# haosulab/ActiveZero

Hardware: AMD Instinct MI355X
Metric: stereo pairs/sec (540x960, D=192) fwd+bwd (higher is better)
Workload: dtype f32; 1 GPU; configs[1]: PSMNet 540x960 (padded to 544 rows) D=192 fwd+bwd+Adam, supervised disparity loss, batch 4 per GPU; global_batch=4, height=540, width=960, maxdisp=192, parallelism=dp1

## Files before the change

activezero_amd/conv3d.py:

```python
import collections
import os

import torch

from . import _lib, overlap, packing, profiler
from .amax import AMAX_SLOTS, ZEROS, absmax, _get_amax, _set_amax, weight_amax
from .handover import slot_contribute, slot_leftover, slot_register, sum_parts
from .ops import _call, _chk, _p, _stream

CONV_S1, CONV_S2, DECONV_S2 = 0, 1, 2
FP32, BF16X6, F16X3 = 0, 1, 3
_PREC = {"fp32": FP32, "bf16x6": BF16X6, "f16x3": F16X3}
_BWD_F16 = os.environ.get("AZ_BWD_F16", "1") != "0"
PRESPLIT = os.environ.get("AZ_PRESPLIT", "1") != "0"
BF16X6_R16 = 2
_ROLL = os.environ.get("AZ_CONV_ROLL", "1") != "0"


_OFF32 = 0xffffff00


def _fits32(x, cin, cout):
    if isinstance(x, LazyCostVolume):
        return True
    _, d, h, w, _ = x.shape
    return d * h * w * max(cin, cout) * 4 < _OFF32


def _fits32_transposed(x, op_cin, op_cout):
    if not (op_cin == 64 and op_cout == 32):
        return True
    _, d, h, w, _ = x.shape
    return d * h * w * 64 * 4 < _OFF32 and 8 * d * h * w * 32 * 4 < _OFF32


def _layout(precision, mode, op_cout, fits32=True):
    if precision == BF16X6 and mode == CONV_S1 and op_cout == 32 and _ROLL and fits32:
        return BF16X6_R16
    return precision


def _fwd_launch(weight, mode):
    if mode == DECONV_S2:
        cin, cout = weight.shape[0], weight.shape[1]
        return cin, cout, 27, cout * 27
    cout, cin = weight.shape[0], weight.shape[1]
    return cin, cout, cin * 27, 27


def _dgrad_launch(mode, cin, cout):
    if mode == CONV_S1:
        return CONV_S1, cout, cin, 27, cin * 27, True
    if mode == CONV_S2:
        return DECONV_S2, cout, cin, 27, cin * 27, False
    return CONV_S2, cout, cin, cout * 27, 27, False


def _f16_fwd_ok(mode, cin, cout):
    return cin in (32, 64) and cout in (32, 64)


def _f16_dgrad_ok(mode, cin, cout):
    return _f16_fwd_ok(*_dgrad_launch(mode, cin, cout)[:3])


def _f16_wgrad_ok(mode, cin, cout):
    return cin in (32, 64) and cout in (32, 64)


def _f16_launch_ok(op_mode, ci, co, operand):
    if not _f16_fwd_ok(op_mode, ci, co):
        return False
    if op_mode == DECONV_S2:
        return _fits32_transposed(operand, ci, co)
    if _fits32(operand, ci, co):
        return True
    if op_mode == CONV_S1:
        return not (co == 32 or ci == co == 64)
    return not (ci == 32 and co == 64 and _lib.lib().az_option(b"AZ_CONV_S2ROLL") != 0)


class Arith(collections.namedtuple("Arith", "conv wgrad sink bwd16", defaults=(None, False))):
    __slots__ = ()

    @classmethod
    def of(cls, conv="bf16x6", wgrad=None, bwd16=None):
        w = wgrad if wgrad is not None else conv
        if bwd16 is None:
            bwd16 = _BWD_F16 or conv == "f16x3"
        return cls(_PREC[conv], BF16X6 if w == "f16x3" else _PREC[w], None, bool(bwd16) and conv != "fp32" and w != "fp32")

    @property
    def names(self):
        inv = {v: k for k, v in _PREC.items()}
        return inv[self.conv], ("f16x3" if self.bwd16 else inv[self.wgrad])


DEFAULT_ARITH = Arith.of(os.environ.get("AZ_CONV_PRECISION", "f16x3"), os.environ.get("AZ_WGRAD_PRECISION"))


def _arith(a):
    if a is None:
        return DEFAULT_ARITH
    if isinstance(a, str):
        return Arith.of(a)
    return a


def _dims(x):
    b, d, h, w, c = x.shape
    return b, d, h, w, c


def _out_dims(mode, d, h, w):
    if mode == CONV_S1:
        return d, h, w
    if mode == CONV_S2:
        return (d - 1) // 2 + 1, (h - 1) // 2 + 1, (w - 1) // 2 + 1
    return 2 * d, 2 * h, 2 * w


def _pack(weight, op_cin, op_cout, stride_out, stride_in, flip, precision, cache=False):
    w = _chk(weight.detach().contiguous(), "weight")

    def make():
        n = _lib.lib().az_conv3d_packed_floats(op_cin, op_cout, precision)
        packed = torch.empty(n, dtype=torch.float32, device=w.device)
        _call("az_conv3d_pack_weights", _p(packed), _p(w), op_cin, op_cout, stride_out, stride_in,
              int(flip), precision, _stream())
        packed.az_precision = precision
        return packed

    key = (packing.cache_key(weight), op_cin, op_cout, stride_out, stride_in, bool(flip), precision) if cache else None
    return packing.memo(packing.PACK_CACHE, key, make, (weight,), 256)


def eval_affine(bn, like, cache=False):
    c = bn.num_features
    src = (bn.weight, bn.bias, bn.running_mean, bn.running_var, bn.num_batches_tracked)

    def make():
        scale, shift = like.new_empty(c), like.new_empty(c)
        _call("az_bn3d_eval_affine", _p(scale), _p(shift), _p(bn.weight.detach()), _p(bn.bias.detach()),
              _p(bn.running_mean), _p(bn.running_var), float(bn.eps), c, _stream())
        return scale, shift

    return packing.memo(packing.AFFINE_CACHE, (packing.cache_key(*src), float(bn.eps)) if cache else None, make, src, 512)


def _pack_forward(weight, mode, precision, cache=False, lazy=False, fits32=True):
    cin, cout, s_out, s_in = _fwd_launch(weight, mode)
    if not lazy:
        precision = _layout(precision, mode, cout, fits32)
    return _pack(weight, cin, cout, s_out, s_in, False, precision, cache), cin, cout


def _peak(precision):
    if precision == F16X3:
        return _PEAK_F16
    return (157.3, "fp32 MFMA") if precision == FP32 else (2500.0 / 6.0, "bf16x6: bf16 MFMA peak / 6")


def _conv_flops(b, vox_out, cin, cout, mode):
    taps = 27.0 / 8.0 if mode == DECONV_S2 else 27.0
    return 2.0 * taps * cin * cout * b * vox_out


class LazyCostVolume:

    def __init__(self, feat_l_nhwc, feat_r_nhwc, ndisp):
        self.fl, self.fr, self.ndisp = _chk(feat_l_nhwc, "feat_l"), _chk(feat_r_nhwc, "feat_r"), int(ndisp)
        if self.fl.shape != self.fr.shape or self.fl.shape[-1] != 32:
            raise RuntimeError("fused cost volume expects two [B,h,w,32] feature maps")


def _run_gather(x, packed, mode, cin, cout, precision, scale=None, shift=None, residual=None, relu=False,
                stats=False, tag="conv3d"):
    if isinstance(x, LazyCostVolume):
        if stats or mode != CONV_S1 or cin != 64:
            raise RuntimeError("the fused cost-volume operand is only wired for the eval-mode dres0[0] conv")
        b, h, w, _ = x.fl.shape
        d = x.ndisp
        out = x.fl.new_empty(b, d, h, w, cout)
        with profiler.scope(f"{tag}_costvol_m0_{cin}_{cout}", flops=_conv_flops(b, d * h * w, cin, cout, mode),
                            peak=_peak(precision)):
            _call("az_conv3d_fwd", _p(out), _p(x.fl), _p(x.fr), _p(packed), _p(scale), _p(shift),
                  _p(residual), int(relu), mode, 1, getattr(packed, "az_precision", precision), b, cin, cout, d, h, w,
                  _stream())
        return out
    b, d, h, w, c = _dims(x)
    assert c == cin, (c, cin)
    precision = getattr(packed, "az_precision", precision)
    if mode == CONV_S2 and ((d % 2 and d != 1) or h % 2 or w % 2):
        raise RuntimeError("stride-2 layers need even D/H/W (as PSMNet's hourglass does; D = 1: a 2-D layer)")
    do, ho, wo = _out_dims(mode, d, h, w)
    out = x.new_empty(b, do, ho, wo, cout)
    flops = _conv_flops(b, do * ho * wo, cin, cout, mode)
    name = f"{tag}_m{mode}_{cin}_{cout}"
    if stats:
        ntiles = _lib.lib().az_conv3d_stats_tiles(mode, precision, b, cin, cout, d, h, w)
        if ntiles <= 0:
            raise RuntimeError(f"az_conv3d_stats_tiles: {ntiles}")
        part = x.new_empty(cout, ntiles, 2)
        cnt = x.new_empty(ntiles)
        with profiler.scope(name, flops=flops, peak=_peak(precision)):
            _call("az_conv3d_fwd_stats", _p(out), _p(part), _p(cnt), _p(x), None, _p(packed), mode, 0,
                  precision, b, cin, cout, d, h, w, _stream())
        return out, part, cnt, ntiles
    with profiler.scope(name, flops=flops, peak=_peak(precision)):
        _call("az_conv3d_fwd", _p(out), _p(x), None, _p(packed), _p(scale), _p(shift), _p(residual),
              int(relu), mode, 0, precision, b, cin, cout, d, h, w, _stream())
    return out


_PEAK_F16 = (2500.0 / 3.0, "f16x3: fp16 MFMA peak / 3")


def _pack_f16(weight, op_cin, op_cout, stride_out, stride_in, flip, mode, cache=False):
    w = _chk(weight.detach().contiguous(), "weight")

    def pack_now(packed, w_amax):
        _call("az_conv3d_pack_weights_f16", _p(packed), _p(w), _p(w_amax), op_cin, op_cout, stride_out, stride_in,
              int(flip), mode, _stream())

    def make():
        w_amax = weight_amax(weight, w)
        packed = torch.empty(_lib.lib().az_conv3d_packed_floats_f16(op_cin, op_cout), dtype=torch.float32, device=w.device)
        pack_now(packed, w_amax)
        return packed, w_amax

    if cache:
        key = (packing.cache_key(weight), op_cin, op_cout, stride_out, stride_in, bool(flip), F16X3, mode)
        return packing.memo(packing.PACK_CACHE, key, make, (weight,), 256)
    kind = _lib.lib().az_conv3d_f16_layout(mode, op_cin, op_cout)
    if kind < 0:
        raise RuntimeError(f"az_conv3d_f16_layout({mode}, {op_cin}, {op_cout}): {kind}")
    hit = packing.planned_pack(weight, w, kind, op_cin, op_cout, op_cin, op_cout, stride_out, stride_in, 27, flip, pack_now)
    return hit if hit is not None else make()


def _is_split(t):
    return getattr(t, "az_split", False)


def _run_f16(x, packed, w_amax, mode, cin, cout, scale=None, shift=None, residual=None, relu=False, stats=False,
             tag="conv3d"):
    b, d, h, w, c = _dims(x)
    assert c == cin, (c, cin)
    do, ho, wo = _out_dims(mode, d, h, w)
    out = x.new_empty(b, do, ho, wo, cout)
    name = f"{tag}_m{mode}_{cin}_{cout}"
    flops = _conv_flops(b, do * ho * wo, cin, cout, mode)
    split = _is_split(x)
    x_amax = _get_amax(x) if split else absmax(x)
    if split and (stats or x_amax is None):
        raise RuntimeError("a pre-split tensor reached a launch that cannot read it")
    if stats:
        ntiles = _lib.lib().az_conv3d_stats_tiles_f16(mode, b, cin, cout, d, h, w)
        if ntiles <= 0:
            raise RuntimeError(f"az_conv3d_stats_tiles_f16: {ntiles}")
        part, cnt = x.new_empty(cout, ntiles, 2), x.new_empty(ntiles)
        with profiler.scope(name, flops=flops, peak=_PEAK_F16):
            _call("az_conv3d_fwd_stats_f16", _p(out), _p(part), _p(cnt), _p(x), _p(packed), _p(x_amax), _p(w_amax),
                  mode, b, cin, cout, d, h, w, _stream())
        return out, part, cnt, ntiles
    with profiler.scope(name, flops=flops, peak=_PEAK_F16):
        _call("az_conv3d_fwd_f16", _p(out), _p(x), _p(packed), _p(x_amax), _p(w_amax), int(split), _p(scale), _p(shift),
              _p(residual), int(relu), mode, b, cin, cout, d, h, w, _stream())
    return out


def _conv(x, weight, mode, precision, scale=None, shift=None, residual=None, relu=False, stats=False, cache=False,
          tag="conv3d"):
    lazy = isinstance(x, LazyCostVolume)
    cin, cout, s_out, s_in = _fwd_launch(weight, mode)
    if precision == F16X3 and not lazy and _f16_launch_ok(mode, cin, cout, x):
        pk, w_amax = _pack_f16(weight, cin, cout, s_out, s_in, False, mode, cache)
        return _run_f16(x, pk, w_amax, mode, cin, cout, scale, shift, residual, relu, stats, tag)
    prec = BF16X6 if precision == F16X3 else precision
    packed, cin, cout = _pack_forward(weight, mode, prec, cache=cache, lazy=lazy, fits32=_fits32(x, cin, cout))
    return _run_gather(x, packed, mode, cin, cout, prec, scale, shift, residual, relu, stats, tag)


def _wgrad_f16(coarse, fine, stride, cm, cn, tag, sink=None, late_ok=True):
    b, dc, hc, wc, _ = _dims(coarse)
    _, df, hf, wf, _ = _dims(fine)
    gw = coarse.new_empty(cm, cn, 3, 3, 3)
    ws_bytes = _lib.lib().az_conv3d_wgrad_workspace(cm, cn)
    am_c, am_f = _get_amax(coarse), _get_amax(fine)
    mask = (1 if _is_split(coarse) else 0) | (2 if _is_split(fine) else 0)
    if (mask & 1 and am_c is None) or (mask & 2 and am_f is None):
        raise RuntimeError("a pre-split tensor without its producer's amax")
    with overlap.scope(sink, coarse, fine, gw, am_c, am_f):
        late = late_ok and sink is not None and sink.live and overlap.DEFER_UNPACK
        ws = sink.take_workspace(ws_bytes // 4) if late else coarse.new_empty(ws_bytes // 4)
        am_c = am_c if mask & 1 else absmax(coarse)
        am_f = am_f if mask & 2 else absmax(fine)
        with profiler.scope(f"{tag}_wgrad_s{stride}_{cm}_{cn}", flops=2.0 * 27 * cm * cn * b * dc * hc * wc,
                            peak=_PEAK_F16):
            _call("az_conv3d_wgrad_f16", None if late else _p(gw), _p(ws), ws_bytes, _p(coarse), _p(fine), _p(am_c), _p(am_f),
                  mask, stride, b, cm, cn, dc, hc, wc, df, hf, wf, _stream())
        if late:
            sink.defer_unpack(gw, ws, cm, cn, cm, cn, 27)
        if sink is not None and sink.live:
            sink.keep.extend((am_c, am_f))
    return gw


def _weight_grad_f16(x, dy, mode, cin, cout, sink=None, late_ok=True):
    if mode == DECONV_S2:
        return _wgrad_f16(x, dy, 2, cin, cout, "deconv", sink, late_ok)
    return _wgrad_f16(dy, x, 1 if mode == CONV_S1 else 2, cout, cin, "conv", sink, late_ok)


def _wgrad(coarse, fine, stride, cm, cn, tag, precision, sink=None):
    b, dc, hc, wc, _ = _dims(coarse)
    _, df, hf, wf, _ = _dims(fine)
    gw = coarse.new_empty(cm, cn, 3, 3, 3)
    ws_bytes = _lib.lib().az_conv3d_wgrad_workspace(cm, cn)
    with overlap.scope(sink, coarse, fine, gw):
        ws = coarse.new_empty(ws_bytes // 4)
        with profiler.scope(f"{tag}_wgrad_s{stride}_{cm}_{cn}", flops=2.0 * 27 * cm * cn * b * dc * hc * wc,
                            peak=_peak(precision)):
            _call("az_conv3d_wgrad", _p(gw), _p(ws), ws_bytes, _p(coarse), _p(fine), stride, precision,
                  b, cm, cn, dc, hc, wc, df, hf, wf, _stream())
    return gw


def _input_grad(dy, weight, mode, cin, cout, precision, residual=None):
    op, ci, co, s_out, s_in, flip = _dgrad_launch(mode, cin, cout)
    if precision == F16X3:
        if _f16_launch_ok(op, ci, co, dy):
            pk, w_amax = _pack_f16(weight, ci, co, s_out, s_in, flip, op)
            return _run_f16(dy, pk, w_amax, op, ci, co, residual=residual, tag="dgrad")
        precision = BF16X6
    pk = _pack(weight, ci, co, s_out, s_in, flip, _layout(precision, op, co, _fits32(dy, ci, co)))
    return _run_gather(dy, pk, op, ci, co, precision, residual=residual, tag="dgrad")


def _weight_grad(x, dy, mode, cin, cout, precision, sink=None, late_ok=True):
    if precision == F16X3:
        if _f16_wgrad_ok(mode, cin, cout):
            return _weight_grad_f16(x, dy, mode, cin, cout, sink, late_ok)
        precision = BF16X6
    if mode == DECONV_S2:
        return _wgrad(x, dy, 2, cin, cout, "deconv", precision, sink)
    return _wgrad(dy, x, 1 if mode == CONV_S1 else 2, cout, cin, "conv", precision, sink)


def _presplit_ok(x, raw, mode, cin, cout, need_gx, need_gw):
    lib = _lib.lib()
    b, d, h, w, _ = raw.shape
    if need_gx:
        op, ci, co = _dgrad_launch(mode, cin, cout)[:3]
        if not _f16_launch_ok(op, ci, co, raw) or lib.az_conv3d_fwd_f16_split_ok(op, b, ci, co, d, h, w) != 1:
            return False
    if need_gw:
        if not _f16_wgrad_ok(mode, cin, cout):
            return False
        _, dx_, hx, wx, _ = x.shape
        if mode == DECONV_S2:
            ok, bit = lib.az_conv3d_wgrad_f16_split_ok(2, b, cin, cout, dx_, hx, wx, d, h, w), 2
        else:
            ok, bit = lib.az_conv3d_wgrad_f16_split_ok(1 if mode == CONV_S1 else 2, b, cout, cin, d, h, w, dx_, hx, wx), 1
        if not ok & bit:
            return False
    return bool(need_gx or need_gw)


class _ConvBN(torch.autograd.Function):

    @staticmethod
    def forward(ctx, x, weight, gamma, beta, residual, bn, mode, relu, arith, defer=None, x_slot=None, res_slot=None):
        ctx.x_slot, ctx.res_slot = x_slot, res_slot
        x = _chk(x, "x")
        if residual is not None:
            residual = _chk(residual, "residual")
        training = bn.training or not bn.track_running_stats
        eps = float(bn.eps)
        cin, cout = _fwd_launch(weight, mode)[:2]
        with torch.cuda.device(x.device):
            if not training:
                scale, shift = eval_affine(bn, x)
                raw = _conv(x, weight, mode, arith.conv)
                y = torch.empty_like(raw)
                y_amax = ZEROS.take(raw)
                _call("az_bn3d_apply", _p(y), _p(raw), _p(scale), _p(shift), _p(residual), int(relu),
                      raw.numel() // cout, cout, _p(y_amax), _stream())
                _set_amax(y, y_amax)
                ctx.save_for_backward(x, weight, gamma, raw, y if relu else None, bn.running_mean.clone(),
                                      scale, None, None)
                ctx.cfg = (mode, relu, residual is not None, cin, cout, arith, False)
                return y
            raw, part, cnt, ntiles = _conv(x, weight, mode, arith.conv, stats=True)
            scale, shift = x.new_empty(cout), x.new_empty(cout)
            mean, invstd = x.new_empty(cout), x.new_empty(cout)
            track = bn.track_running_stats and bn.running_mean is not None
            momentum = 0.1 if bn.momentum is None else float(bn.momentum)
            nbt = bn.num_batches_tracked if (track and bn.num_batches_tracked is not None) else None
            scratch = x.new_empty(int(_lib.lib().az_bn3d_finalize_scratch(cout))) if ntiles >= 4096 else None
            _call("az_bn3d_finalize", _p(mean), _p(invstd), _p(scale), _p(shift),
                  _p(bn.running_mean) if track else None, _p(bn.running_var) if track else None,
                  _p(part), _p(cnt), _p(gamma.detach()), _p(beta.detach()), ntiles, cout, eps,
                  momentum, _p(nbt), _p(scratch), scratch.numel() if scratch is not None else 0, _stream())
            if nbt is not None:
                packing.touched(nbt, bn.running_mean, bn.running_var)
            nvox = raw.numel() // cout
            if defer is not None and relu and residual is None:
                defer.scale, defer.shift = scale, shift
                y = raw
            else:
                y = torch.empty_like(raw)
                y_amax = ZEROS.take(raw)
                with profiler.scope(f"bn3d_apply_{cout}", bytes=4.0 * raw.numel() * (3 if residual is not None else 2),
                                    bound="hbm"):
                    _call("az_bn3d_apply", _p(y), _p(raw), _p(scale), _p(shift), _p(residual), int(relu),
                          nvox, cout, _p(y_amax), _stream())
                _set_amax(y, y_amax)
        remask = relu and residual is None
        ctx.save_for_backward(x, weight, gamma, raw, y if (relu and not remask) else None, mean, invstd,
                              scale if remask else None, shift if remask else None)
        if arith.sink is not None and not arith.sink.owns(weight):
            arith = arith._replace(sink=None)
        ctx.cfg = (mode, relu, residual is not None, cin, cout, arith, True)
        ctx.x_amax = _get_amax(x)
        return y

    @staticmethod
    def backward(ctx, gy):
        x, weight, gamma, raw, y, mean, invstd, scale, shift = ctx.saved_tensors
        mode, relu, has_res, cin, cout, arith, training = ctx.cfg
        gy = _chk(gy.contiguous(), "grad_y")
        nvox = raw.numel() // cout
        with torch.cuda.device(gy.device):
            gy = slot_leftover(ctx, gy)
            if not training:
                s_, rm = invstd, mean
                dz = gy * (y > 0).to(gy.dtype) if relu else gy
                dbeta = dz.sum(dim=(0, 1, 2, 3))
                rinv = torch.where(gamma.detach() != 0, s_ / gamma.detach(), torch.zeros_like(s_))
                dgamma = (dz * (raw - rm)).sum(dim=(0, 1, 2, 3)) * rinv
                dx_raw = (dz * s_).contiguous()
                g_res = dz if has_res else None
            else:
                lib = _lib.lib()
                dx_raw = torch.empty_like(raw)
                dz = torch.empty_like(raw) if (has_res and relu) else None
                dgamma, dbeta = gy.new_empty(cout), gy.new_empty(cout)
                coef = gy.new_empty(cout, 3)
                ws_bytes = lib.az_bn3d_bwd_workspace(nvox, cout)
                ws = gy.new_empty(ws_bytes // 4)
                dx_amax = gy.new_empty(AMAX_SLOTS) if arith.bwd16 else None
                split = arith.bwd16 and PRESPLIT and _presplit_ok(x, raw, mode, cin, cout, ctx.needs_input_grad[0],
                                                                  ctx.needs_input_grad[1])
                with profiler.scope(f"bn3d_bwd_{cout}", bytes=4.0 * raw.numel() * (7 if (relu and y is not None) else 5), bound="hbm"):
                    _call("az_bn3d_bwd", _p(dx_raw), _p(dz), _p(dgamma), _p(dbeta), _p(coef), _p(ws), ws_bytes,
                          _p(gy), _p(y), _p(raw), _p(mean), _p(invstd), _p(gamma.detach()), _p(scale), _p(shift),
                          int(relu), nvox, cout, _p(dx_amax), int(split), _stream())
                if dx_amax is not None:
                    _set_amax(dx_raw, dx_amax)
                if split:
                    dx_raw.az_split = True
                g_res = (dz if relu else gy) if has_res else None
            gx = gw = None
            if has_res:
                g_res = slot_contribute(ctx.res_slot, plain=g_res)
            if ctx.needs_input_grad[0]:
                gx = slot_contribute(ctx.x_slot, make=lambda r: _input_grad(dx_raw, weight, mode, cin, cout,
                                                                             F16X3 if arith.bwd16 else arith.conv, r))
            if ctx.needs_input_grad[1]:
                if getattr(ctx, "x_amax", None) is not None and _get_amax(x) is None:
                    _set_amax(x, ctx.x_amax)
                gw = _weight_grad(x, dx_raw, mode, cin, cout, F16X3 if arith.bwd16 else arith.wgrad, arith.sink)
        return gx, gw, dgamma, dbeta, g_res, None, None, None, None, None, None, None


class DeferredAffine:

    def __init__(self):
        self.scale = self.shift = None

    @property
    def pending(self):
        return self.scale is not None


def conv_bn(x, conv, bn, mode, relu=False, residual=None, arith=None, defer=None):
    arith = _arith(arith)
    if isinstance(x, LazyCostVolume):
        if torch.is_grad_enabled() or bn.training:
            raise RuntimeError("LazyCostVolume is an inference-only operand")
        with torch.cuda.device(x.fl.device):
            scale, shift = eval_affine(bn, x.fl, cache=True)
            return _conv(x, conv.weight, mode, arith.conv, scale, shift, residual, relu, cache=True)
    training = bn.training or not bn.track_running_stats
    if not training and not torch.is_grad_enabled():
        x = _chk(x, "x")
        with torch.cuda.device(x.device):
            scale, shift = eval_affine(bn, x, cache=True)
            return _conv(x, conv.weight, mode, arith.conv, scale, shift,
                         _chk(residual, "residual") if residual is not None else None, relu, cache=True)
    w = arith.sink.weight(conv.weight) if arith.sink is not None else conv.weight
    x_slot = slot_register(x)
    res_slot = slot_register(residual) if residual is not None else None
    return _ConvBN.apply(x, w, bn.weight, bn.bias, residual, bn, mode, relu, arith, defer, x_slot, res_slot)


class _ConvLogits(torch.autograd.Function):

    @staticmethod
    def forward(ctx, x, weight, addend, sink, scale=None, shift=None):
        ctx.sink = sink if (sink is not None and sink.owns(weight)) else None
        x = _chk(x, "x")
        w = _chk(weight.detach().contiguous(), "weight")
        b, d, h, wd, c = _dims(x)
        if c != 32 or tuple(w.shape) != (1, 32, 3, 3, 3):
            raise RuntimeError("classifier conv expects 32 -> 1 channels, 3x3x3")
        if addend is not None:
            addend = _chk(addend.contiguous(), "addend")
        out = x.new_empty(b, d, h, wd)
        with torch.cuda.device(x.device):
            with profiler.scope("conv3d_c1_fwd", bytes=4.0 * (x.numel() + out.numel()), bound="hbm"):
                _call("az_conv3d_c1_fwd", _p(out), _p(x), _p(w), _p(addend), _p(scale), _p(shift), b, d, h, wd, _stream())
        ctx.save_for_backward(x, w, scale, shift)
        ctx.has_add = addend is not None
        return out

    @staticmethod
    def backward(ctx, g):
        x, w, scale, shift = ctx.saved_tensors
        g = _chk(g.contiguous(), "grad_logits")
        b, d, h, wd, _ = _dims(x)
        gx = gw = None
        with torch.cuda.device(g.device):
            if ctx.needs_input_grad[0]:
                gx = torch.empty_like(x)
                with profiler.scope("conv3d_c1_dgrad", bytes=4.0 * (x.numel() + g.numel()), bound="hbm"):
                    _call("az_conv3d_c1_dgrad", _p(gx), _p(g), _p(w), b, d, h, wd, _stream())
            if ctx.needs_input_grad[1]:
                gw = torch.empty_like(w)
                with overlap.scope(ctx.sink, x, g, gw, scale, shift), \
                        profiler.scope("conv3d_c1_wgrad", bytes=4.0 * (x.numel() + g.numel()), bound="hbm"):
                    _call("az_conv3d_c1_wgrad", _p(gw), _p(x), _p(g), _p(scale), _p(shift), b, d, h, wd, _stream())
        return gx, gw, (g if ctx.has_add else None), None, None, None


def conv_logits(x, conv, addend=None, sink=None, affine=None):
    sc, sh = (affine.scale, affine.shift) if (affine is not None and affine.pending) else (None, None)
    return _ConvLogits.apply(x, sink.weight(conv.weight) if sink is not None else conv.weight, addend, sink, sc, sh)


class _AddRelu(torch.autograd.Function):
    @staticmethod
    def forward(ctx, a, b):
        a, b = _chk(a, "a"), _chk(b, "b")
        y = torch.empty_like(a)
        y_amax = ZEROS.take(a)
        with torch.cuda.device(a.device):
            _call("az_add_relu", _p(y), _p(a), _p(b), 0, a.numel(), _p(y_amax), _stream())
        _set_amax(y, y_amax)
        return y

    @staticmethod
    def backward(ctx, g):
        return g, g


def add(a, b):
    return _AddRelu.apply(a, b)


class _FanOut(torch.autograd.Function):

    @staticmethod
    def forward(ctx, x, n):
        views = tuple(x.view_as(x) for _ in range(n))
        am = _get_amax(x)
        if am is not None:
            for v in views:
                _set_amax(v, am)
        return views

    @staticmethod
    def backward(ctx, *grads):
        gs = [_chk(g.contiguous(), "grad") for g in grads if g is not None]
        if not gs:
            return None, None
        with torch.cuda.device(gs[0].device):
            return sum_parts(gs), None


def fanout(x, n):
    if not (torch.is_grad_enabled() and x.requires_grad) or x.numel() % 4:
        return (x,) * n
    return _FanOut.apply(x, n)


def conv_plain(x, weight, mode, arith=None):
    arith = _arith(arith)
    return _conv(_chk(x, "x"), weight, mode, arith.conv)
```

activezero_amd/csrc/az_bn3d.hip:

```cpp
#include <stdlib.h>

#include "az_roll_common.h"

__device__ __forceinline__ double bn_wave_sum(double v) {
#pragma unroll
    for (int o = 32; o > 0; o >>= 1) v += __shfl_xor(v, o);
    return v;
}
template <int NT>
__device__ __forceinline__ double bn_block_sum(double v, double *slots ) {
    v = bn_wave_sum(v);
    __syncthreads();
    if ((threadIdx.x & 63) == 0) slots[threadIdx.x >> 6] = v;
    __syncthreads();
    double t = 0.0;
#pragma unroll
    for (int w = 0; w < NT / 64; ++w) t += slots[w];
    return t;
}

#define BN_PRE_SLICES 32
__global__ void __launch_bounds__(256)
bn_premerge_kernel(float *__restrict__ part_out, float *__restrict__ cnt_out, const float *__restrict__ part,
                   const float *__restrict__ cnt, long long ntiles) {
    const int c = blockIdx.x, sl = blockIdx.y;
    const long long per = (ntiles + BN_PRE_SLICES - 1) / BN_PRE_SLICES;
    const long long t0 = sl * per, t1 = t0 + per < ntiles ? t0 + per : ntiles;
    __shared__ double slots[256 / 64];
    const float2 *pc = reinterpret_cast<const float2 *>(part) + (long long)c * ntiles;
    double n = 0.0, sum = 0.0;
    for (long long t = t0 + threadIdx.x; t < t1; t += 256) {
        n += (double)cnt[t];
        sum += (double)pc[t].x;
    }
    const double N = bn_block_sum<256>(n, slots);
    const double S = bn_block_sum<256>(sum, slots);
    const double mean = N > 0.0 ? S / N : 0.0;
    double m2 = 0.0;
    for (long long t = t0 + threadIdx.x; t < t1; t += 256) {
        const float nt = cnt[t];
        if (nt <= 0.f) continue;
        const float2 pr = pc[t];
        const double dlt = (double)pr.x / (double)nt - mean;
        m2 += (double)pr.y + (double)nt * dlt * dlt;
    }
    const double M2 = bn_block_sum<256>(m2, slots);
    if (threadIdx.x == 0) {
        reinterpret_cast<float2 *>(part_out)[c * BN_PRE_SLICES + sl] = make_float2((float)S, (float)M2);
        if (c == 0) cnt_out[sl] = (float)N;
    }
}

#define BN_FIN_THREADS 1024
__global__ void __launch_bounds__(BN_FIN_THREADS)
bn_finalize_kernel(float *__restrict__ mean_out, float *__restrict__ invstd_out,
                   float *__restrict__ scale, float *__restrict__ shift,
                   float *__restrict__ running_mean, float *__restrict__ running_var,
                   const float *__restrict__ part, const float *__restrict__ cnt,
                   const float *__restrict__ gamma, const float *__restrict__ beta,
                   long long ntiles, int C, float eps, float momentum, int groups,
                   long long *__restrict__ num_batches_tracked) {
    const int c = blockIdx.x;
    if (num_batches_tracked != nullptr && c == 0 && threadIdx.x == 0) *num_batches_tracked += groups;
    for (int grp = 0; grp < groups; ++grp, part += (long long)C * ntiles * 2, cnt += ntiles,
             mean_out += C, invstd_out += C, scale += C, shift += C) {
    __shared__ double slots[BN_FIN_THREADS / 64];
    const float2 *pc = reinterpret_cast<const float2 *>(part) + (long long)c * ntiles;
    double n = 0.0, sum = 0.0;
    for (long long t = threadIdx.x; t < ntiles; t += BN_FIN_THREADS) {
        n += (double)cnt[t];
        sum += (double)pc[t].x;
    }
    const double Ntot = bn_block_sum<BN_FIN_THREADS>(n, slots);
    const double mean_all = bn_block_sum<BN_FIN_THREADS>(sum, slots) / Ntot;
    double m2 = 0.0;
    for (long long t = threadIdx.x; t < ntiles; t += BN_FIN_THREADS) {
        const float nt = cnt[t];
        if (nt <= 0.f) continue;
        const float2 pr = pc[t];
        const double dlt = (double)pr.x / (double)nt - mean_all;
        m2 += (double)pr.y + (double)nt * dlt * dlt;
    }
    const double M2 = bn_block_sum<BN_FIN_THREADS>(m2, slots);
    if (threadIdx.x == 0) {
        const double N = Ntot, mu = mean_all, var = M2 / N;
        const double istd = 1.0 / sqrt(var + (double)eps);
        mean_out[c] = (float)mu;
        invstd_out[c] = (float)istd;
        const float sc = gamma[c] * (float)istd;
        scale[c] = sc;
        shift[c] = beta[c] - (float)mu * sc;
        if (running_mean) {
            const double unbiased = N > 1.0 ? M2 / (N - 1.0) : var;
            running_mean[c] = (1.f - momentum) * running_mean[c] + momentum * (float)mu;
            running_var[c] = (1.f - momentum) * running_var[c] + momentum * (float)unbiased;
        }
    }
    }
}

__global__ void bn_eval_affine_kernel(float *scale, float *shift, const float *gamma,
                                      const float *beta, const float *rm, const float *rv,
                                      float eps, int C) {
    const int c = blockIdx.x * blockDim.x + threadIdx.x;
    if (c >= C) return;
    const float sc = gamma[c] / sqrtf(rv[c] + eps);
    scale[c] = sc;
    shift[c] = beta[c] - rm[c] * sc;
}

typedef float az_v4f __attribute__((ext_vector_type(4)));
template <bool NT>
__device__ __forceinline__ float4 bn_ld4(const float4 *p) {
    if (NT) {
        const az_v4f v = __builtin_nontemporal_load(reinterpret_cast<const az_v4f *>(p));
        return make_float4(v[0], v[1], v[2], v[3]);
    }
    return *p;
}
template <bool NT>
__device__ __forceinline__ void bn_st4(float4 *p, const float4 &o) {
    if (NT) {
        const az_v4f v = {o.x, o.y, o.z, o.w};
        __builtin_nontemporal_store(v, reinterpret_cast<az_v4f *>(p));
    } else {
        *p = o;
    }
}
#define BN_NT_BYTES (256LL << 20)

template <int C, bool NT>
__global__ void __launch_bounds__(256)
bn_apply_kernel(float4 *__restrict__ y, const float4 *__restrict__ x,
                const float *__restrict__ scale, const float *__restrict__ shift,
                const float4 *__restrict__ res, int relu, long long total4, unsigned *__restrict__ amax = nullptr) {
    constexpr int C4 = C / 4;
    unsigned am = 0;
    __shared__ float4 ssc[C4], ssh[C4];
    {
        const long long go = (long long)blockIdx.y * total4;
        y += go; x += go; if (res) res += go;
        scale += blockIdx.y * C; shift += blockIdx.y * C;
    }
    if (threadIdx.x < C4) {
        ssc[threadIdx.x] = reinterpret_cast<const float4 *>(scale)[threadIdx.x];
        ssh[threadIdx.x] = reinterpret_cast<const float4 *>(shift)[threadIdx.x];
    }
    __syncthreads();
    for (long long i = blockIdx.x * 256LL + threadIdx.x; i < total4; i += gridDim.x * 256LL) {
        const int c4 = (int)(i % C4);
        const float4 v = bn_ld4<NT>(&x[i]), sc = ssc[c4], sh = ssh[c4];
        float4 o = make_float4(fmaf(v.x, sc.x, sh.x), fmaf(v.y, sc.y, sh.y), fmaf(v.z, sc.z, sh.z),
                               fmaf(v.w, sc.w, sh.w));
        if (res) {
            const float4 r = bn_ld4<NT>(&res[i]);
            o.x += r.x; o.y += r.y; o.z += r.z; o.w += r.w;
        }
        if (relu) {
            o.x = fmaxf(o.x, 0.f); o.y = fmaxf(o.y, 0.f); o.z = fmaxf(o.z, 0.f); o.w = fmaxf(o.w, 0.f);
        }
        bn_st4<NT>(&y[i], o);
        az_amax_acc(am, o);
    }
    if (amax) az_amax_flush(amax, am);
}

__device__ __forceinline__ int c4_of(int tid, int C4) { return tid % C4; }

template <int C, bool NT>
__global__ void __launch_bounds__(256)
bn_bwd_reduce_kernel(float *__restrict__ partial, const float *__restrict__ dy,
                     const float *__restrict__ y, const float *__restrict__ x,
                     const float *__restrict__ mean, const float *__restrict__ invstd,
                     const float *__restrict__ scale, const float *__restrict__ shift, int relu,
                     long long nvox, unsigned *__restrict__ amax_zero = nullptr, unsigned *__restrict__ pmax = nullptr) {
    if (amax_zero && blockIdx.x == 0 && blockIdx.y == 0 && threadIdx.x < AZ_AMAX_SLOTS) amax_zero[threadIdx.x * AZ_AMAX_STRIDE] = 0u;
    constexpr int C4 = C / 4, VPB = 256 / C4;
    const bool remask = relu && scale != nullptr;
    {
        const long long go = (long long)blockIdx.y * nvox * C;
        dy += go; x += go; if (relu && !remask) y += go;
        mean += blockIdx.y * C; invstd += blockIdx.y * C;
        if (remask) { scale += blockIdx.y * C; shift += blockIdx.y * C; }
        partial += (size_t)blockIdx.y * gridDim.x * C * 2;
    }
    float4 sc = make_float4(0, 0, 0, 0), sh = sc;
    if (remask) { sc = reinterpret_cast<const float4 *>(scale)[c4_of(threadIdx.x, C4)]; sh = reinterpret_cast<const float4 *>(shift)[c4_of(threadIdx.x, C4)]; }
    const int c4 = threadIdx.x % C4, vl = threadIdx.x / C4;
    const float4 mu = reinterpret_cast<const float4 *>(mean)[c4];
    const float4 is = reinterpret_cast<const float4 *>(invstd)[c4];
    float4 s1 = make_float4(0, 0, 0, 0), s2 = make_float4(0, 0, 0, 0);
    uint4 mg = make_uint4(0, 0, 0, 0), mx = make_uint4(0, 0, 0, 0);
    auto body = [&](const float4 gin, const float4 xx, const float4 yin, float4 &t1, float4 &t2) {
        float4 g = gin;
        if (relu) {
            float4 yy = yin;
            if (remask) yy = make_float4(fmaf(xx.x, sc.x, sh.x), fmaf(xx.y, sc.y, sh.y), fmaf(xx.z, sc.z, sh.z), fmaf(xx.w, sc.w, sh.w));
            g.x = yy.x > 0.f ? g.x : 0.f; g.y = yy.y > 0.f ? g.y : 0.f;
            g.z = yy.z > 0.f ? g.z : 0.f; g.w = yy.w > 0.f ? g.w : 0.f;
        }
        const float4 xh = make_float4((xx.x - mu.x) * is.x, (xx.y - mu.y) * is.y, (xx.z - mu.z) * is.z, (xx.w - mu.w) * is.w);
        t1.x += g.x; t1.y += g.y; t1.z += g.z; t1.w += g.w;
        t2.x += g.x * xh.x; t2.y += g.y * xh.y; t2.z += g.z * xh.z; t2.w += g.w * xh.w;
        if (pmax) {
            mg.x = max(mg.x, az_finite_abs_bits(g.x)); mg.y = max(mg.y, az_finite_abs_bits(g.y));
            mg.z = max(mg.z, az_finite_abs_bits(g.z)); mg.w = max(mg.w, az_finite_abs_bits(g.w));
            mx.x = max(mx.x, az_finite_abs_bits(xh.x)); mx.y = max(mx.y, az_finite_abs_bits(xh.y));
            mx.z = max(mx.z, az_finite_abs_bits(xh.z)); mx.w = max(mx.w, az_finite_abs_bits(xh.w));
        }
    };
    const long long stride = (long long)gridDim.x * VPB;
    float4 u1 = make_float4(0, 0, 0, 0), u2 = make_float4(0, 0, 0, 0);
    const float4 zero4 = make_float4(0, 0, 0, 0);
    long long v = (long long)blockIdx.x * VPB + vl;
    for (; v + stride < nvox; v += 2 * stride) {
        const size_t i = (size_t)v * C4 + c4, i2 = (size_t)(v + stride) * C4 + c4;
        const float4 ga = bn_ld4<NT>(reinterpret_cast<const float4 *>(dy) + i), gb = bn_ld4<NT>(reinterpret_cast<const float4 *>(dy) + i2);
        const float4 xa = bn_ld4<NT>(reinterpret_cast<const float4 *>(x) + i), xb = bn_ld4<NT>(reinterpret_cast<const float4 *>(x) + i2);
        float4 ya = zero4, yb = zero4;
        if (relu && !remask) { ya = bn_ld4<NT>(reinterpret_cast<const float4 *>(y) + i); yb = bn_ld4<NT>(reinterpret_cast<const float4 *>(y) + i2); }
        body(ga, xa, ya, s1, s2);
        body(gb, xb, yb, u1, u2);
    }
    if (v < nvox) {
        const size_t i = (size_t)v * C4 + c4;
        const float4 ga = bn_ld4<NT>(reinterpret_cast<const float4 *>(dy) + i), xa = bn_ld4<NT>(reinterpret_cast<const float4 *>(x) + i);
        float4 ya = zero4;
        if (relu && !remask) ya = bn_ld4<NT>(reinterpret_cast<const float4 *>(y) + i);
        body(ga, xa, ya, s1, s2);
    }
    s1.x += u1.x; s1.y += u1.y; s1.z += u1.z; s1.w += u1.w;
    s2.x += u2.x; s2.y += u2.y; s2.z += u2.z; s2.w += u2.w;
    static_assert(C4 <= 64 && 64 % C4 == 0, "channel quads must tile a wave");
#pragma unroll
    for (int off = C4; off < 64; off <<= 1) {
        s1.x += __shfl_xor(s1.x, off); s1.y += __shfl_xor(s1.y, off); s1.z += __shfl_xor(s1.z, off); s1.w += __shfl_xor(s1.w, off);
        s2.x += __shfl_xor(s2.x, off); s2.y += __shfl_xor(s2.y, off); s2.z += __shfl_xor(s2.z, off); s2.w += __shfl_xor(s2.w, off);
    }
    __shared__ float4 r1[4][C4], r2[4][C4];
    const int wave = threadIdx.x >> 6, lane = threadIdx.x & 63;
    if (lane < C4) { r1[wave][lane] = s1; r2[wave][lane] = s2; }
    __syncthreads();
    if (threadIdx.x < C4) {
#pragma unroll
        for (int k = 1; k < 4; ++k) {
            const float4 a = r1[k][c4], b = r2[k][c4];
            s1.x += a.x; s1.y += a.y; s1.z += a.z; s1.w += a.w;
            s2.x += b.x; s2.y += b.y; s2.z += b.z; s2.w += b.w;
        }
        float *p = partial + ((size_t)blockIdx.x * C + c4 * 4) * 2;
        p[0] = s1.x; p[1] = s2.x; p[2] = s1.y; p[3] = s2.y;
        p[4] = s1.z; p[5] = s2.z; p[6] = s1.w; p[7] = s2.w;
    }
    if (pmax) {
#pragma unroll
        for (int off = C4; off < 64; off <<= 1) {
            mg.x = max(mg.x, (unsigned)__shfl_xor((int)mg.x, off)); mg.y = max(mg.y, (unsigned)__shfl_xor((int)mg.y, off));
            mg.z = max(mg.z, (unsigned)__shfl_xor((int)mg.z, off)); mg.w = max(mg.w, (unsigned)__shfl_xor((int)mg.w, off));
            mx.x = max(mx.x, (unsigned)__shfl_xor((int)mx.x, off)); mx.y = max(mx.y, (unsigned)__shfl_xor((int)mx.y, off));
            mx.z = max(mx.z, (unsigned)__shfl_xor((int)mx.z, off)); mx.w = max(mx.w, (unsigned)__shfl_xor((int)mx.w, off));
        }
        __shared__ uint4 q1[4][C4], q2[4][C4];
        if (lane < C4) { q1[wave][lane] = mg; q2[wave][lane] = mx; }
        __syncthreads();
        if (threadIdx.x < C4) {
#pragma unroll
            for (int k = 1; k < 4; ++k) {
                const uint4 a = q1[k][c4], b = q2[k][c4];
                mg.x = max(mg.x, a.x); mg.y = max(mg.y, a.y); mg.z = max(mg.z, a.z); mg.w = max(mg.w, a.w);
                mx.x = max(mx.x, b.x); mx.y = max(mx.y, b.y); mx.z = max(mx.z, b.z); mx.w = max(mx.w, b.w);
            }
            unsigned *p = pmax + ((size_t)blockIdx.y * gridDim.x * C + (size_t)blockIdx.x * C + c4 * 4) * 2;
            p[0] = mg.x; p[1] = mx.x; p[2] = mg.y; p[3] = mx.y;
            p[4] = mg.z; p[5] = mx.z; p[6] = mg.w; p[7] = mx.w;
        }
    }
}

#define BN_BWD_PARTIAL_FLOATS 32768
template <int C, bool NT>
__global__ void __launch_bounds__(256)
bn_bwd_apply_kernel(float4 *__restrict__ dx, float4 *__restrict__ dz_out,
                    const float4 *__restrict__ dy, const float4 *__restrict__ y,
                    const float4 *__restrict__ x, const float *__restrict__ mean,
                    const float *__restrict__ invstd, float *__restrict__ coef,
                    const float *__restrict__ scale, const float *__restrict__ shift, int relu,
                    long long total4, const float *__restrict__ partial, int nblocks, const float *__restrict__ gamma,
                    float *__restrict__ dgamma, float *__restrict__ dbeta, double nvox,
                    unsigned *__restrict__ amax = nullptr, const unsigned *__restrict__ pmax = nullptr) {
    constexpr int C4 = C / 4;
    unsigned am = 0;
    float split_scale = 1.f;
    __shared__ float smu[C], sis[C], k0[C], k1[C], k2[C], ssc[C], ssh[C];
    const bool remask = relu && scale != nullptr;
    const int grp = blockIdx.y;
    {
        const long long go = (long long)grp * total4;
        dx += go; dy += go; x += go; if (relu && !remask) y += go; if (dz_out) dz_out += go;
        mean += grp * C; invstd += grp * C; coef += grp * C * 3;
        if (remask) { scale += grp * C; shift += grp * C; }
    }
    if (remask && threadIdx.x < C) { ssc[threadIdx.x] = scale[threadIdx.x]; ssh[threadIdx.x] = shift[threadIdx.x]; }
    if (threadIdx.x < C) {
        smu[threadIdx.x] = mean[threadIdx.x];
        sis[threadIdx.x] = invstd[threadIdx.x];
    }
    constexpr int COLS = C / 2, ROWS = 256 / COLS;
    static_assert(COLS <= 64 && 64 % COLS == 0, "a partial row must tile a wave");
    __shared__ float wsum[4][2 * C];
    const int j = threadIdx.x % COLS, r = threadIdx.x / COLS, wave = threadIdx.x >> 6;
    const bool writer = blockIdx.x == 0;
    const int g_lo = (writer && grp == 0) ? 0 : grp, g_hi = (writer && grp == 0) ? (int)gridDim.y : grp + 1;
    double dg_tot = 0.0, db_tot = 0.0;
    for (int g = g_lo; g < g_hi; ++g) {
        const float4 *p4 = reinterpret_cast<const float4 *>(partial) + (size_t)g * nblocks * COLS;
        double a0 = 0.0, a1 = 0.0, a2 = 0.0, a3 = 0.0;
        for (int blk = r; blk < nblocks; blk += ROWS) {
            const float4 v = p4[(size_t)blk * COLS + j];
            a0 += v.x; a1 += v.y; a2 += v.z; a3 += v.w;
        }
#pragma unroll
        for (int off = COLS; off < 64; off <<= 1) {
            a0 += __shfl_xor(a0, off); a1 += __shfl_xor(a1, off); a2 += __shfl_xor(a2, off); a3 += __shfl_xor(a3, off);
        }
        __syncthreads();
        if ((threadIdx.x & 63) < COLS) {
            wsum[wave][4 * j + 0] = (float)a0; wsum[wave][4 * j + 1] = (float)a1;
            wsum[wave][4 * j + 2] = (float)a2; wsum[wave][4 * j + 3] = (float)a3;
        }
        __syncthreads();
        if (threadIdx.x < C) {
            const int c = threadIdx.x;
            const double sa = ((double)wsum[0][2 * c] + (double)wsum[1][2 * c]) + ((double)wsum[2][2 * c] + (double)wsum[3][2 * c]);
            const double sb = ((double)wsum[0][2 * c + 1] + (double)wsum[1][2 * c + 1]) + ((double)wsum[2][2 * c + 1] + (double)wsum[3][2 * c + 1]);
            db_tot += sa; dg_tot += sb;
            if (g == grp) {
                k0[c] = gamma[c] * sis[c];
                k1[c] = (float)(sa / nvox);
                k2[c] = (float)(sb / nvox);
                if (writer) { coef[c * 3 + 0] = k0[c]; coef[c * 3 + 1] = k1[c]; coef[c * 3 + 2] = k2[c]; }
            }
        }
    }
    if (writer && grp == 0 && threadIdx.x < C) { dbeta[threadIdx.x] = (float)db_tot; dgamma[threadIdx.x] = (float)dg_tot; }
    if (pmax) {
        const uint4 *m4 = reinterpret_cast<const uint4 *>(pmax);
        uint4 m = make_uint4(0, 0, 0, 0);
        for (int blk = r; blk < nblocks; blk += ROWS) {
            const uint4 v = m4[(size_t)blk * COLS + j];
            m.x = max(m.x, v.x); m.y = max(m.y, v.y); m.z = max(m.z, v.z); m.w = max(m.w, v.w);
        }
#pragma unroll
        for (int off = COLS; off < 64; off <<= 1) {
            m.x = max(m.x, (unsigned)__shfl_xor((int)m.x, off)); m.y = max(m.y, (unsigned)__shfl_xor((int)m.y, off));
            m.z = max(m.z, (unsigned)__shfl_xor((int)m.z, off)); m.w = max(m.w, (unsigned)__shfl_xor((int)m.w, off));
        }
        __syncthreads();
        if ((threadIdx.x & 63) < COLS) {
            wsum[wave][4 * j + 0] = __uint_as_float(m.x); wsum[wave][4 * j + 1] = __uint_as_float(m.y);
            wsum[wave][4 * j + 2] = __uint_as_float(m.z); wsum[wave][4 * j + 3] = __uint_as_float(m.w);
        }
        __syncthreads();
        float bnd = 0.f;
        if (threadIdx.x < C) {
            const int c = threadIdx.x;
            const float gm = fmaxf(fmaxf(wsum[0][2 * c], wsum[1][2 * c]), fmaxf(wsum[2][2 * c], wsum[3][2 * c]));
            const float xm = fmaxf(fmaxf(wsum[0][2 * c + 1], wsum[1][2 * c + 1]), fmaxf(wsum[2][2 * c + 1], wsum[3][2 * c + 1]));
            bnd = fabsf(k0[c]) * (gm + fabsf(k1[c]) + xm * fabsf(k2[c])) * 1.000001f;
            bnd = bnd < __builtin_inff() ? bnd : 0.f;
        }
#pragma unroll
        for (int off = 32; off > 0; off >>= 1) bnd = fmaxf(bnd, __shfl_xor(bnd, off));
        __shared__ float bwave[4];
        if ((threadIdx.x & 63) == 0) bwave[wave] = bnd;
        __syncthreads();
        bnd = fmaxf(fmaxf(bwave[0], bwave[1]), fmaxf(bwave[2], bwave[3]));
        split_scale = az_pow2(az_f16_scale_exp(bnd));
        if (writer && grp == 0 && threadIdx.x == 0 && amax) amax[0] = __float_as_uint(bnd);
    }
    __syncthreads();
    for (long long i = blockIdx.x * 256LL + threadIdx.x; i < total4; i += gridDim.x * 256LL) {
        const int c = (int)(i % C4) * 4;
        float4 g = bn_ld4<NT>(&dy[i]);
        const float4 xx = bn_ld4<NT>(&x[i]);
        if (relu) {
            float4 yy;
            if (remask) yy = make_float4(fmaf(xx.x, ssc[c + 0], ssh[c + 0]), fmaf(xx.y, ssc[c + 1], ssh[c + 1]),
                                         fmaf(xx.z, ssc[c + 2], ssh[c + 2]), fmaf(xx.w, ssc[c + 3], ssh[c + 3]));
            else yy = bn_ld4<NT>(&y[i]);
            g.x = yy.x > 0.f ? g.x : 0.f; g.y = yy.y > 0.f ? g.y : 0.f;
            g.z = yy.z > 0.f ? g.z : 0.f; g.w = yy.w > 0.f ? g.w : 0.f;
        }
        if (dz_out) bn_st4<NT>(&dz_out[i], g);
        float4 o;
        o.x = k0[c + 0] * (g.x - k1[c + 0] - (xx.x - smu[c + 0]) * sis[c + 0] * k2[c + 0]);
        o.y = k0[c + 1] * (g.y - k1[c + 1] - (xx.y - smu[c + 1]) * sis[c + 1] * k2[c + 1]);
        o.z = k0[c + 2] * (g.z - k1[c + 2] - (xx.z - smu[c + 2]) * sis[c + 2] * k2[c + 2]);
        o.w = k0[c + 3] * (g.w - k1[c + 3] - (xx.w - smu[c + 3]) * sis[c + 3] * k2[c + 3]);
        if (pmax) {
            bn_st4<NT>(&dx[i], az_presplit_f16x4(make_float4(o.x * split_scale, o.y * split_scale, o.z * split_scale, o.w * split_scale)));
        } else {
            bn_st4<NT>(&dx[i], o);
            az_amax_acc(am, o);
        }
    }
    if (amax && !pmax) az_amax_flush(amax, am);
}

__global__ void __launch_bounds__(256)
add_relu_kernel(float4 *__restrict__ y, const float4 *__restrict__ a,
                const float4 *__restrict__ b, int relu, long long total4, unsigned *__restrict__ amax) {
    unsigned am = 0;
    for (long long i = blockIdx.x * 256LL + threadIdx.x; i < total4; i += gridDim.x * 256LL) {
        const float4 p = a[i], q = b[i];
        float4 o = make_float4(p.x + q.x, p.y + q.y, p.z + q.z, p.w + q.w);
        if (relu) {
            o.x = fmaxf(o.x, 0.f); o.y = fmaxf(o.y, 0.f); o.z = fmaxf(o.z, 0.f); o.w = fmaxf(o.w, 0.f);
        }
        y[i] = o;
        az_amax_acc(am, o);
    }
    if (amax) az_amax_flush(amax, am);
}


template <int C>
__global__ void __launch_bounds__(256)
bn_stats_kernel(float *__restrict__ part, float *__restrict__ cnt, const float *__restrict__ x,
                long long nvox, long long ntiles) {
    constexpr int C4 = C / 4, VPB = 256 / C4;
    const int c4 = threadIdx.x % C4, vl = threadIdx.x / C4;
    x += (size_t)blockIdx.y * nvox * C;
    part += (size_t)blockIdx.y * C * ntiles * 2;
    cnt += (size_t)blockIdx.y * ntiles;
    const long long v0 = (long long)blockIdx.x * VPB;
    const float4 K = reinterpret_cast<const float4 *>(x)[(size_t)v0 * C4 + c4];
    float4 s1 = make_float4(0, 0, 0, 0), s2 = make_float4(0, 0, 0, 0);
    int n = 0;
    for (long long v = v0 + vl; v < nvox; v += (long long)gridDim.x * VPB) {
        const float4 a = reinterpret_cast<const float4 *>(x)[(size_t)v * C4 + c4];
        const float dx = a.x - K.x, dy = a.y - K.y, dz = a.z - K.z, dw = a.w - K.w;
        s1.x += dx; s1.y += dy; s1.z += dz; s1.w += dw;
        s2.x += dx * dx; s2.y += dy * dy; s2.z += dz * dz; s2.w += dw * dw;
        ++n;
    }
    __shared__ float4 r1[256], r2[256];
    __shared__ int rn[256];
    r1[threadIdx.x] = s1; r2[threadIdx.x] = s2; rn[threadIdx.x] = n;
    __syncthreads();
    if (vl == 0) {
        for (int k = 1; k < VPB; ++k) {
            const float4 a = r1[k * C4 + c4], b = r2[k * C4 + c4];
            s1.x += a.x; s1.y += a.y; s1.z += a.z; s1.w += a.w;
            s2.x += b.x; s2.y += b.y; s2.z += b.z; s2.w += b.w;
            n += rn[k * C4 + c4];
        }
        const float fn = (float)n;
        const float s[4] = {s1.x, s1.y, s1.z, s1.w}, q[4] = {s2.x, s2.y, s2.z, s2.w};
        const float k4[4] = {K.x, K.y, K.z, K.w};
#pragma unroll
        for (int e = 0; e < 4; ++e) {
            float2 o;
            o.x = s[e] + fn * k4[e];
            o.y = fmaxf(q[e] - s[e] * s[e] / fn, 0.f);
            reinterpret_cast<float2 *>(part)[(size_t)(c4 * 4 + e) * ntiles + blockIdx.x] = o;
        }
        if (c4 == 0) cnt[blockIdx.x] = fn;
    }
}

__global__ void __launch_bounds__(256)
sum4_kernel(float4 *__restrict__ y, const float4 *__restrict__ a, const float4 *__restrict__ b,
            const float4 *__restrict__ c, const float4 *__restrict__ d, long long total4) {
    for (long long i = blockIdx.x * 256LL + threadIdx.x; i < total4; i += gridDim.x * 256LL) {
        const float4 p = a[i], q = b[i];
        float4 o = make_float4(p.x + q.x, p.y + q.y, p.z + q.z, p.w + q.w);
        if (c) { const float4 r = c[i]; o.x += r.x; o.y += r.y; o.z += r.z; o.w += r.w; }
        if (d) { const float4 r = d[i]; o.x += r.x; o.y += r.y; o.z += r.z; o.w += r.w; }
        y[i] = o;
    }
}

#define BN_GRID(total) az_grid_for((total), 256)
static int bn_bwd_fused_blocks(int blocks, int C) {
    const int cap = BN_BWD_PARTIAL_FLOATS / (2 * C);
    return blocks < cap ? blocks : cap;
}
static unsigned bn_bwd_apply_grid(long long total4) {
    const unsigned g = az_grid_for(total4, 256);
    return g < 1024u ? g : 1024u;
}
#define BN_LAUNCH(KERNEL, C, NT, GRID, STREAM, ...)                                                             \
    do {                                                                                                        \
        if (NT) {                                                                                               \
            if ((C) == 32) hipLaunchKernelGGL((KERNEL<32, true>), GRID, dim3(256), 0, STREAM, __VA_ARGS__);     \
            else if ((C) == 64) hipLaunchKernelGGL((KERNEL<64, true>), GRID, dim3(256), 0, STREAM, __VA_ARGS__); \
            else hipLaunchKernelGGL((KERNEL<128, true>), GRID, dim3(256), 0, STREAM, __VA_ARGS__);              \
        } else {                                                                                                \
            if ((C) == 32) hipLaunchKernelGGL((KERNEL<32, false>), GRID, dim3(256), 0, STREAM, __VA_ARGS__);    \
            else if ((C) == 64) hipLaunchKernelGGL((KERNEL<64, false>), GRID, dim3(256), 0, STREAM, __VA_ARGS__); \
            else hipLaunchKernelGGL((KERNEL<128, false>), GRID, dim3(256), 0, STREAM, __VA_ARGS__);             \
        }                                                                                                       \
    } while (0)

extern "C" long long az_bn3d_finalize_scratch(int C) { return (long long)C * BN_PRE_SLICES * 2 + BN_PRE_SLICES; }

extern "C" int az_bn3d_finalize(float *mean, float *invstd, float *scale, float *shift,
                                float *running_mean, float *running_var, const float *partials,
                                const float *counts, const float *gamma, const float *beta,
                                long long ntiles, int C, float eps, float momentum,
                                long long *num_batches_tracked, float *scratch,
                                long long scratch_floats, void *stream) {
    AZ_REQUIRE_PTR(mean); AZ_REQUIRE_PTR(invstd); AZ_REQUIRE_PTR(scale); AZ_REQUIRE_PTR(shift);
    AZ_REQUIRE_PTR(partials); AZ_REQUIRE_PTR(counts); AZ_REQUIRE_PTR(gamma); AZ_REQUIRE_PTR(beta);
    AZ_REQUIRE(ntiles > 0 && C > 0);
    if ((running_mean == nullptr) != (running_var == nullptr)) return AZ_EINVAL;
    if (scratch != nullptr && ntiles >= 4096) {
        if (scratch_floats < az_bn3d_finalize_scratch(C)) return AZ_EWORKSPACE;
        float *p2 = scratch, *c2 = scratch + (size_t)C * BN_PRE_SLICES * 2;
        hipLaunchKernelGGL(bn_premerge_kernel, dim3(C, BN_PRE_SLICES), dim3(256), 0, az_stream(stream), p2, c2, partials,
                           counts, ntiles);
        partials = p2; counts = c2; ntiles = BN_PRE_SLICES;
    }
    hipLaunchKernelGGL(bn_finalize_kernel, dim3(C), dim3(BN_FIN_THREADS), 0, az_stream(stream), mean, invstd,
                       scale, shift, running_mean, running_var, partials, counts, gamma, beta,
                       ntiles, C, eps, momentum, 1, num_batches_tracked);
    return az_launch_status();
}

extern "C" int az_bn3d_eval_affine(float *scale, float *shift, const float *gamma,
                                   const float *beta, const float *running_mean,
                                   const float *running_var, float eps, int C, void *stream) {
    AZ_REQUIRE_PTR(scale); AZ_REQUIRE_PTR(shift); AZ_REQUIRE_PTR(gamma); AZ_REQUIRE_PTR(beta);
    AZ_REQUIRE_PTR(running_mean); AZ_REQUIRE_PTR(running_var);
    AZ_REQUIRE(C > 0);
    hipLaunchKernelGGL(bn_eval_affine_kernel, dim3((C + 63) / 64), dim3(64), 0, az_stream(stream),
                       scale, shift, gamma, beta, running_mean, running_var, eps, C);
    return az_launch_status();
}

extern "C" int az_bn3d_apply(float *y, const float *x, const float *scale, const float *shift,
                             const float *residual, int relu, long long nvox, int C, float *y_amax,
                             void *stream) {
    AZ_REQUIRE_PTR(y); AZ_REQUIRE_PTR(x); AZ_REQUIRE_PTR(scale); AZ_REQUIRE_PTR(shift);
    AZ_REQUIRE(nvox > 0);
    const long long total4 = nvox * C / 4;
    const float4 *r4 = reinterpret_cast<const float4 *>(residual);
    if (C != 32 && C != 64 && C != 128) return AZ_EUNSUPPORTED;
    const bool nt = total4 * 16 >= BN_NT_BYTES;
    BN_LAUNCH(bn_apply_kernel, C, nt, dim3(BN_GRID(total4)), az_stream(stream), (float4 *)y, (const float4 *)x, scale,
              shift, r4, relu, total4, reinterpret_cast<unsigned *>(y_amax));
    return az_launch_status();
}

static long long bn3d_bwd_blocks(long long nvox, int C) {
    const int vpb = 256 / (C / 4);
    return az_grid_for((nvox + vpb - 1) / vpb * 256, 256);
}
extern "C" long long az_bn3d_bwd_workspace(long long nvox, int C) {
    if (nvox <= 0 || (C != 32 && C != 64 && C != 128)) return AZ_EINVAL;
    return 2 * bn3d_bwd_blocks(nvox, C) * C * 2 * (long long)sizeof(float);
}

extern "C" int az_bn3d_bwd(float *dx, float *dz_out, float *dgamma, float *dbeta, float *coef,
                           float *workspace, long long workspace_bytes, const float *dy,
                           const float *y, const float *x, const float *mean,
                           const float *invstd, const float *gamma, const float *scale,
                           const float *shift, int relu, long long nvox, int C, float *dx_amax, int split_out,
                           void *stream) {
    unsigned *const am = reinterpret_cast<unsigned *>(dx_amax);
    AZ_REQUIRE_PTR(dx); AZ_REQUIRE_PTR(dgamma); AZ_REQUIRE_PTR(dbeta); AZ_REQUIRE_PTR(coef);
    AZ_REQUIRE_PTR(workspace); AZ_REQUIRE_PTR(dy); AZ_REQUIRE_PTR(x); AZ_REQUIRE_PTR(mean);
    AZ_REQUIRE_PTR(invstd); AZ_REQUIRE_PTR(gamma);
    if ((scale == nullptr) != (shift == nullptr)) return AZ_EINVAL;
    if (relu && !scale) AZ_REQUIRE_PTR(y);
    const long long need = az_bn3d_bwd_workspace(nvox, C);
    if (need < 0) return (int)need;
    if (workspace_bytes < need) return AZ_EWORKSPACE;
    int blocks = (int)bn3d_bwd_blocks(nvox, C);
    const long long total4 = nvox * C / 4;
    hipStream_t s = az_stream(stream);
    const bool nt = total4 * 16 >= BN_NT_BYTES;
    if (split_out && !am) return AZ_ENULL;
    blocks = bn_bwd_fused_blocks(blocks, C);
    unsigned *const pmax = split_out ? reinterpret_cast<unsigned *>(workspace) + (size_t)blocks * C * 2 : nullptr;
    BN_LAUNCH(bn_bwd_reduce_kernel, C, nt, dim3(blocks), s, workspace, dy, y, x, mean, invstd, scale, shift, relu, nvox, am, pmax);
    BN_LAUNCH(bn_bwd_apply_kernel, C, nt, dim3(bn_bwd_apply_grid(total4)), s, (float4 *)dx, (float4 *)dz_out, (const float4 *)dy,
              (const float4 *)y, (const float4 *)x, mean, invstd, coef, scale, shift, relu, total4,
              (const float *)workspace, blocks, gamma, dgamma, dbeta, (double)nvox, am, (const unsigned *)pmax);
    return az_launch_status();
}

extern "C" int az_add_relu(float *y, const float *a, const float *b, int relu, long long n, float *y_amax,
                           void *stream) {
    AZ_REQUIRE_PTR(y); AZ_REQUIRE_PTR(a); AZ_REQUIRE_PTR(b);
    AZ_REQUIRE(n > 0 && n % 4 == 0);
    hipLaunchKernelGGL(add_relu_kernel, dim3(BN_GRID(n / 4)), dim3(256), 0, az_stream(stream),
                       (float4 *)y, (const float4 *)a, (const float4 *)b, relu, n / 4, reinterpret_cast<unsigned *>(y_amax));
    return az_launch_status();
}

extern "C" int az_sum4(float *y, const float *a, const float *b, const float *c, const float *d, long long n,
                       void *stream) {
    AZ_REQUIRE_PTR(y); AZ_REQUIRE_PTR(a); AZ_REQUIRE_PTR(b);
    if (d && !c) return AZ_EINVAL;
    AZ_REQUIRE(n > 0 && n % 4 == 0);
    hipLaunchKernelGGL(sum4_kernel, dim3(BN_GRID(n / 4)), dim3(256), 0, az_stream(stream), (float4 *)y,
                       (const float4 *)a, (const float4 *)b, (const float4 *)c, (const float4 *)d, n / 4);
    return az_launch_status();
}

extern "C" long long az_bn3d_stats_tiles(long long nvox, int C) {
    if (nvox <= 0 || (C != 32 && C != 64 && C != 128)) return AZ_EINVAL;
    const int vpb = 256 / (C / 4);
    long long t = (nvox + (long long)vpb * 16 - 1) / ((long long)vpb * 16);
    if (t > 2048) t = 2048;
    if (t < 1) t = 1;
    return t;
}

extern "C" int az_bn3d_stats(float *partials, float *counts, const float *x, long long nvox, int C,
                             void *stream) {
    AZ_REQUIRE_PTR(partials); AZ_REQUIRE_PTR(counts); AZ_REQUIRE_PTR(x);
    const long long tiles = az_bn3d_stats_tiles(nvox, C);
    if (tiles < 0) return (int)tiles;
    hipStream_t s = az_stream(stream);
    if (C == 32)
        hipLaunchKernelGGL(bn_stats_kernel<32>, dim3((unsigned)tiles), dim3(256), 0, s, partials, counts, x, nvox, tiles);
    else if (C == 64)
        hipLaunchKernelGGL(bn_stats_kernel<64>, dim3((unsigned)tiles), dim3(256), 0, s, partials, counts, x, nvox, tiles);
    else
        hipLaunchKernelGGL(bn_stats_kernel<128>, dim3((unsigned)tiles), dim3(256), 0, s, partials, counts, x, nvox, tiles);
    return az_launch_status();
}

static int bn2d_blocks(long long nvox, int C) {
    const int vpb = 256 / (C / 4);
    return (int)az_grid_for((nvox + vpb - 1) / vpb * 256, 256);
}

extern "C" long long az_bn2d_workspace(int groups, long long nvox, int C) {
    const long long tiles = az_bn3d_stats_tiles(nvox, C);
    if (tiles < 0 || groups <= 0) return AZ_EINVAL;
    const long long fwd = (long long)groups * (C * tiles * 2 + tiles);
    const long long bwd = (long long)groups * ((long long)bn2d_blocks(nvox, C) * C * 2 + C * 3);
    return (fwd > bwd ? fwd : bwd) * (long long)sizeof(float);
}

template <int C>
static void bn2d_fwd_launch(float *y, float *mean, float *invstd, float *scale, float *shift, float *rm,
                            float *rv, const float *x, const float *res, const float *gamma,
                            const float *beta, float *ws, int relu, int groups, long long nvox, float eps,
                            float momentum, long long *nbt, const float *pre_part, const float *pre_cnt,
                            long long pre_tiles, hipStream_t s, unsigned *amax) {
    long long tiles = az_bn3d_stats_tiles(nvox, C);
    const float *part = ws, *cnt = ws + (size_t)groups * C * tiles * 2;
    if (pre_part != nullptr) {
        part = pre_part; cnt = pre_cnt; tiles = pre_tiles;
    } else {
        hipLaunchKernelGGL(bn_stats_kernel<C>, dim3((unsigned)tiles, groups), dim3(256), 0, s, ws,
                           ws + (size_t)groups * C * tiles * 2, x, nvox, tiles);
    }
    hipLaunchKernelGGL(bn_finalize_kernel, dim3(C), dim3(BN_FIN_THREADS), 0, s, mean, invstd, scale, shift, rm, rv,
                       part, cnt, gamma, beta, tiles, C, eps, momentum, groups, nbt);
    const long long total4 = nvox * C / 4;
    hipLaunchKernelGGL((bn_apply_kernel<C, false>), dim3(BN_GRID(total4), groups), dim3(256), 0, s, (float4 *)y,
                       (const float4 *)x, scale, shift, (const float4 *)res, relu, total4, amax);
}

extern "C" int az_bn2d_fwd(float *y, float *mean, float *invstd, float *scale, float *shift,
                           float *running_mean, float *running_var, const float *x, const float *residual,
                           const float *gamma, const float *beta, float *workspace, long long workspace_bytes,
                           int relu, int groups, long long nvox, int C, float eps, float momentum,
                           long long *num_batches_tracked, const float *partials,
                           const float *counts, long long partial_tiles, float *y_amax, void *stream) {
    unsigned *const am = reinterpret_cast<unsigned *>(y_amax);
    AZ_REQUIRE_PTR(y); AZ_REQUIRE_PTR(mean); AZ_REQUIRE_PTR(invstd); AZ_REQUIRE_PTR(scale); AZ_REQUIRE_PTR(shift);
    AZ_REQUIRE_PTR(x); AZ_REQUIRE_PTR(gamma); AZ_REQUIRE_PTR(beta); AZ_REQUIRE_PTR(workspace);
    if ((running_mean == nullptr) != (running_var == nullptr)) return AZ_EINVAL;
    if ((partials == nullptr) != (counts == nullptr) || (partials != nullptr && partial_tiles <= 0)) return AZ_EINVAL;
    const long long need = az_bn2d_workspace(groups, nvox, C);
    if (need < 0) return (int)need;
    if (workspace_bytes < need) return AZ_EWORKSPACE;
    if (groups > 65535) return AZ_EUNSUPPORTED;
    hipStream_t s = az_stream(stream);
    if (C == 32) bn2d_fwd_launch<32>(y, mean, invstd, scale, shift, running_mean, running_var, x, residual, gamma, beta, workspace, relu, groups, nvox, eps, momentum, num_batches_tracked, partials, counts, partial_tiles, s, am);
    else if (C == 64) bn2d_fwd_launch<64>(y, mean, invstd, scale, shift, running_mean, running_var, x, residual, gamma, beta, workspace, relu, groups, nvox, eps, momentum, num_batches_tracked, partials, counts, partial_tiles, s, am);
    else bn2d_fwd_launch<128>(y, mean, invstd, scale, shift, running_mean, running_var, x, residual, gamma, beta, workspace, relu, groups, nvox, eps, momentum, num_batches_tracked, partials, counts, partial_tiles, s, am);
    return az_launch_status();
}

template <int C>
static void bn2d_bwd_launch(float *dx, float *dz, float *dgamma, float *dbeta, float *ws, const float *dy,
                            const float *y, const float *x, const float *mean, const float *invstd,
                            const float *gamma, const float *scale, const float *shift, int relu, int groups,
                            long long nvox, hipStream_t s, unsigned *amax) {
    int blocks = bn2d_blocks(nvox, C);
    float *partial = ws, *coef = ws + (size_t)groups * blocks * C * 2;
    const long long total4 = nvox * C / 4;
    blocks = bn_bwd_fused_blocks(blocks, C);
    hipLaunchKernelGGL((bn_bwd_reduce_kernel<C, false>), dim3(blocks, groups), dim3(256), 0, s, partial, dy, y, x, mean,
                       invstd, scale, shift, relu, nvox);
    hipLaunchKernelGGL((bn_bwd_apply_kernel<C, false>), dim3(bn_bwd_apply_grid(total4), groups), dim3(256), 0, s, (float4 *)dx,
                       (float4 *)dz, (const float4 *)dy, (const float4 *)y, (const float4 *)x, mean, invstd,
                       coef, scale, shift, relu, total4, (const float *)partial, blocks, gamma, dgamma, dbeta, (double)nvox, amax);
}

extern "C" int az_bn2d_bwd(float *dx, float *dz_out, float *dgamma, float *dbeta, float *workspace,
                           long long workspace_bytes, const float *dy, const float *y, const float *x,
                           const float *mean, const float *invstd, const float *gamma, const float *scale,
                           const float *shift, int relu, int groups, long long nvox, int C, float *dx_amax,
                           void *stream) {
    AZ_REQUIRE_PTR(dx); AZ_REQUIRE_PTR(dgamma); AZ_REQUIRE_PTR(dbeta); AZ_REQUIRE_PTR(workspace);
    AZ_REQUIRE_PTR(dy); AZ_REQUIRE_PTR(x); AZ_REQUIRE_PTR(mean); AZ_REQUIRE_PTR(invstd); AZ_REQUIRE_PTR(gamma);
    if ((scale == nullptr) != (shift == nullptr)) return AZ_EINVAL;
    if (relu && !scale) AZ_REQUIRE_PTR(y);
    unsigned *const am = reinterpret_cast<unsigned *>(dx_amax);
    const long long need = az_bn2d_workspace(groups, nvox, C);
    if (need < 0) return (int)need;
    if (workspace_bytes < need) return AZ_EWORKSPACE;
    if (groups > 65535) return AZ_EUNSUPPORTED;
    hipStream_t s = az_stream(stream);
    if (C == 32) bn2d_bwd_launch<32>(dx, dz_out, dgamma, dbeta, workspace, dy, y, x, mean, invstd, gamma, scale, shift, relu, groups, nvox, s, am);
    else if (C == 64) bn2d_bwd_launch<64>(dx, dz_out, dgamma, dbeta, workspace, dy, y, x, mean, invstd, gamma, scale, shift, relu, groups, nvox, s, am);
    else bn2d_bwd_launch<128>(dx, dz_out, dgamma, dbeta, workspace, dy, y, x, mean, invstd, gamma, scale, shift, relu, groups, nvox, s, am);
    return az_launch_status();
}
```

activezero_amd/csrc/az_conv3d_c1.hip:

```cpp
#include "az_common.h"
#include "az_launch_math.h"

#define C1_TH 8
#define C1_TW 32
#define C1_VS 36
#define C1_GP 36
typedef float c1_f2 __attribute__((ext_vector_type(2)));
#define C1_FMA2(a, b, c) __builtin_elementwise_fma(a, b, c)


#define C1F_TH 8
#define C1F_TW 16
template <int CTRL>
__device__ __forceinline__ float c1_dpp_add(float v) {
    return v + __builtin_bit_cast(float, __builtin_amdgcn_update_dpp(0, __builtin_bit_cast(int, v), CTRL, 0xf, 0xf, true));
}
__global__ void __launch_bounds__(256)
c1_fwd_kernel(float *__restrict__ out, const float *__restrict__ in, const float *__restrict__ w,
              const float *__restrict__ addend, const float *__restrict__ in_scale,
              const float *__restrict__ in_shift, int D, int H, int W, int tiles_x, int dseg) {
    constexpr int SX = C1F_TW + 2, SY = C1F_TH + 2;
    __shared__ __attribute__((aligned(16))) float slab[SY * SX * C1_VS];
    const int tx0 = (blockIdx.x % tiles_x) * C1F_TW, ty0 = (blockIdx.x / tiles_x) * C1F_TH;
    const int d0 = blockIdx.y * dseg, d1 = min(d0 + dseg, D), b = blockIdx.z;
    const int cp = threadIdx.x & 15, grp = threadIdx.x >> 4;
    const int ly = grp >> 1, lx0 = (grp & 1) * 8;
    const int oh = ty0 + ly;
    c1_f2 wp[27];
#pragma unroll
    for (int t = 0; t < 27; ++t) wp[t] = c1_f2{w[(cp * 2 + 0) * 27 + t], w[(cp * 2 + 1) * 27 + t]};
    c1_f2 a_prev[8], a_cur[8], a_next[8];
#pragma unroll
    for (int j = 0; j < 8; ++j) { a_prev[j] = c1_f2{0.f, 0.f}; a_cur[j] = c1_f2{0.f, 0.f}; a_next[j] = c1_f2{0.f, 0.f}; }
    constexpr int NQ = SY * SX * 8, NLD = (NQ + 255) / 256;
    float4 pre[NLD];
    const bool affine = in_scale != nullptr;
    float4 isc = make_float4(1.f, 1.f, 1.f, 1.f), ish = make_float4(0.f, 0.f, 0.f, 0.f);
    if (affine) {
        isc = reinterpret_cast<const float4 *>(in_scale)[threadIdx.x & 7];
        ish = reinterpret_cast<const float4 *>(in_shift)[threadIdx.x & 7];
    }
    unsigned okbits = 0;
    auto issue = [&](int id) {
        okbits = 0;
#pragma unroll
        for (int it = 0; it < NLD; ++it) {
            const int q = threadIdx.x + 256 * it, v = q >> 3, part = q & 7;
            const int sy = v / SX, sx = v - sy * SX;
            const int ih = ty0 - 1 + sy, iw = tx0 - 1 + sx;
            pre[it] = make_float4(0.f, 0.f, 0.f, 0.f);
            if (q < NQ && id >= 0 && id < D && ih >= 0 && ih < H && iw >= 0 && iw < W) {
                pre[it] = *reinterpret_cast<const float4 *>(
                    in + ((((size_t)b * D + id) * H + ih) * W + iw) * 32 + part * 4);
                okbits |= 1u << it;
            }
        }
    };
    issue(d0 - 1);
    for (int id = d0 - 1; id <= d1; ++id) {
        if (id >= 0 && id < D) {
            __syncthreads();
#pragma unroll
            for (int it = 0; it < NLD; ++it) {
                const int q = threadIdx.x + 256 * it;
                float4 v = pre[it];
                if (affine && ((okbits >> it) & 1u)) {
                    v.x = fmaxf(fmaf(v.x, isc.x, ish.x), 0.f); v.y = fmaxf(fmaf(v.y, isc.y, ish.y), 0.f);
                    v.z = fmaxf(fmaf(v.z, isc.z, ish.z), 0.f); v.w = fmaxf(fmaf(v.w, isc.w, ish.w), 0.f);
                }
                if (q < NQ) *reinterpret_cast<float4 *>(&slab[(q >> 3) * C1_VS + (q & 7) * 4]) = v;
            }
            __syncthreads();
        }
        if (id < d1) issue(id + 1);
        if (id >= 0 && id < D) {
#pragma unroll
            for (int kh = 0; kh < 3; ++kh) {
                c1_f2 r[10];
                const float *row = &slab[((ly + kh) * SX + lx0) * C1_VS + cp * 2];
#pragma unroll
                for (int i = 0; i < 10; ++i) {
                    const float2 x = *reinterpret_cast<const float2 *>(row + i * C1_VS);
                    r[i] = c1_f2{x.x, x.y};
                }
#pragma unroll
                for (int kw = 0; kw < 3; ++kw)
#pragma unroll
                    for (int j = 0; j < 8; ++j) {
                        a_next[j] = C1_FMA2(r[j + kw], wp[kh * 3 + kw], a_next[j]);
                        a_cur[j] = C1_FMA2(r[j + kw], wp[9 + kh * 3 + kw], a_cur[j]);
                        a_prev[j] = C1_FMA2(r[j + kw], wp[18 + kh * 3 + kw], a_prev[j]);
                    }
            }
        }
        const int od = id - 1;
        if (od >= d0 && od < d1) {
            float mine = 0.f;
#pragma unroll
            for (int j = 0; j < 8; ++j) {
                float v = a_prev[j][0] + a_prev[j][1];
                v = c1_dpp_add<0xB1>(v);
                v = c1_dpp_add<0x4E>(v);
                v = c1_dpp_add<0x141>(v);
                v = c1_dpp_add<0x140>(v);
                mine = (cp == j) ? v : mine;
            }
            const int ow = tx0 + lx0 + cp;
            if (cp < 8 && oh < H && ow < W) {
                const size_t o = (((size_t)b * D + od) * H + oh) * W + ow;
                out[o] = addend ? mine + addend[o] : mine;
            }
        }
#pragma unroll
        for (int j = 0; j < 8; ++j) { a_prev[j] = a_cur[j]; a_cur[j] = a_next[j]; a_next[j] = c1_f2{0.f, 0.f}; }
    }
}

__device__ __forceinline__ void c1_load_gtile(float *gt, const float *__restrict__ gout, int b,
                                              int od, int ty0, int tx0, int D, int H, int W) {
    constexpr int SX = C1_TW + 2, SY = C1_TH + 2;
    for (int q = threadIdx.x; q < 3 * SY * SX; q += 256) {
        const int sx = q % SX;
        const int r = q / SX;
        const int sy = r % SY, sd = r / SY;
        const int gd = od - 1 + sd, gh = ty0 - 1 + sy, gw = tx0 - 1 + sx;
        gt[r * C1_GP + sx] = (gd >= 0 && gd < D && gh >= 0 && gh < H && gw >= 0 && gw < W)
                                 ? gout[(((size_t)b * D + gd) * H + gh) * W + gw] : 0.f;
    }
}
__device__ __forceinline__ void c1_row6(float (&r)[6], const float *gt, int pd, int sy, int lx0) {
    const float *row = static_cast<const float *>(__builtin_assume_aligned(gt + (pd * (C1_TH + 2) + sy) * C1_GP + lx0, 16));
    const float4 a = *reinterpret_cast<const float4 *>(row);
    const float2 c = *reinterpret_cast<const float2 *>(row + 4);
    r[0] = a.x; r[1] = a.y; r[2] = a.z; r[3] = a.w; r[4] = c.x; r[5] = c.y;
}

__global__ void __launch_bounds__(256)
c1_dgrad_kernel(float *__restrict__ gin, const float *__restrict__ gout,
                const float *__restrict__ w, int D, int H, int W, int tiles_x) {
    constexpr int SY = C1_TH + 2;
    __shared__ __attribute__((aligned(16))) float gt[3 * SY * C1_GP];
    const int tx0 = (blockIdx.x % tiles_x) * C1_TW, ty0 = (blockIdx.x / tiles_x) * C1_TH;
    const int od = blockIdx.y, b = blockIdx.z;
    c1_load_gtile(gt, gout, b, od, ty0, tx0, D, H, W);
    const int cp = threadIdx.x & 15, grp = threadIdx.x >> 4;
    c1_f2 wp[27];
#pragma unroll
    for (int t = 0; t < 27; ++t) wp[t] = c1_f2{w[(cp * 2 + 0) * 27 + t], w[(cp * 2 + 1) * 27 + t]};
    __syncthreads();
#pragma unroll 1
    for (int p = 0; p < C1_TH * C1_TW / 128; ++p) {
        const int gi = p * 16 + grp, ly = gi >> 2, lx0 = (gi & 3) * 8;
        const int oh = ty0 + ly;
        c1_f2 acc[8];
#pragma unroll
        for (int j = 0; j < 8; ++j) acc[j] = c1_f2{0.f, 0.f};
#pragma unroll
        for (int kd = 0; kd < 3; ++kd)
#pragma unroll
            for (int kh = 0; kh < 3; ++kh) {
                float r[12];
                {
                    const float *row = static_cast<const float *>(__builtin_assume_aligned(
                        gt + ((2 - kd) * SY + ly + 2 - kh) * C1_GP + lx0, 16));
                    const float4 a = *reinterpret_cast<const float4 *>(row);
                    const float4 c = *reinterpret_cast<const float4 *>(row + 4);
                    const float2 e = *reinterpret_cast<const float2 *>(row + 8);
                    r[0] = a.x; r[1] = a.y; r[2] = a.z; r[3] = a.w; r[4] = c.x; r[5] = c.y; r[6] = c.z; r[7] = c.w;
                    r[8] = e.x; r[9] = e.y;
                }
#pragma unroll
                for (int kw = 0; kw < 3; ++kw) {
                    const int t = (kd * 3 + kh) * 3 + kw;
#pragma unroll
                    for (int j = 0; j < 8; ++j) {
                        const c1_f2 g2 = {r[j + 2 - kw], r[j + 2 - kw]};
                        acc[j] = C1_FMA2(g2, wp[t], acc[j]);
                    }
                }
            }
#pragma unroll
        for (int j = 0; j < 8; ++j) asm volatile("" : "+v"(acc[j]));
        if (oh < H) {
            float *dst = gin + ((((size_t)b * D + od) * H + oh) * W + tx0 + lx0) * 32 + cp * 2;
#pragma unroll
            for (int j = 0; j < 8; ++j)
                if (tx0 + lx0 + j < W) *reinterpret_cast<float2 *>(dst + j * 32) = make_float2(acc[j][0], acc[j][1]);
        }
    }
}

__global__ void __launch_bounds__(256)
c1_wgrad_kernel(float *__restrict__ gw, const float *__restrict__ in,
                const float *__restrict__ gout, const float *__restrict__ in_scale,
                const float *__restrict__ in_shift, int D, int H, int W, int tiles_x, int tiles_y,
                long long ntiles) {
    constexpr int SY = C1_TH + 2;
    __shared__ __attribute__((aligned(16))) float gt[3 * SY * C1_GP];
    __shared__ float red[864];
    for (int q = threadIdx.x; q < 864; q += 256) red[q] = 0.f;
    const int quad = threadIdx.x & 7, grp = threadIdx.x >> 3;
    const bool affine = in_scale != nullptr;
    float4 isc = make_float4(1.f, 1.f, 1.f, 1.f), ish = make_float4(0.f, 0.f, 0.f, 0.f);
    if (affine) {
        isc = reinterpret_cast<const float4 *>(in_scale)[quad];
        ish = reinterpret_cast<const float4 *>(in_shift)[quad];
    }
    c1_f2 a01[27], a23[27];
#pragma unroll
    for (int t = 0; t < 27; ++t) { a01[t] = c1_f2{0.f, 0.f}; a23[t] = c1_f2{0.f, 0.f}; }
    for (long long item = blockIdx.x; item < ntiles; item += gridDim.x) {
        long long r = item;
        const int tx0 = (int)(r % tiles_x) * C1_TW; r /= tiles_x;
        const int ty0 = (int)(r % tiles_y) * C1_TH; r /= tiles_y;
        const int od = (int)(r % D);
        const int b = (int)(r / D);
        __syncthreads();
        c1_load_gtile(gt, gout, b, od, ty0, tx0, D, H, W);
        __syncthreads();
#pragma unroll 1
        for (int p = 0; p < C1_TH * C1_TW / 128; ++p) {
            const int gi = p * 32 + grp, ly = gi >> 3, lx0 = (gi & 7) * 4;
            const int ih = ty0 + ly;
            c1_f2 x01[4], x23[4];
            const float *src = in + ((((size_t)b * D + od) * H + ih) * W + tx0 + lx0) * 32 + quad * 4;
#pragma unroll
            for (int j = 0; j < 4; ++j) {
                float4 x = make_float4(0.f, 0.f, 0.f, 0.f);
                if (ih < H && tx0 + lx0 + j < W) {
                    x = *reinterpret_cast<const float4 *>(src + j * 32);
                    if (affine) {
                        x.x = fmaxf(fmaf(x.x, isc.x, ish.x), 0.f); x.y = fmaxf(fmaf(x.y, isc.y, ish.y), 0.f);
                        x.z = fmaxf(fmaf(x.z, isc.z, ish.z), 0.f); x.w = fmaxf(fmaf(x.w, isc.w, ish.w), 0.f);
                    }
                }
                x01[j] = c1_f2{x.x, x.y}; x23[j] = c1_f2{x.z, x.w};
            }
#pragma unroll
            for (int kd = 0; kd < 3; ++kd)
#pragma unroll
                for (int kh = 0; kh < 3; ++kh) {
                    float r[6];
                    c1_row6(r, gt, 2 - kd, ly + 2 - kh, lx0);
#pragma unroll
                    for (int kw = 0; kw < 3; ++kw) {
                        const int t = (kd * 3 + kh) * 3 + kw;
#pragma unroll
                        for (int j = 0; j < 4; ++j) {
                            const c1_f2 g2 = {r[j + 2 - kw], r[j + 2 - kw]};
                            a01[t] = C1_FMA2(g2, x01[j], a01[t]);
                            a23[t] = C1_FMA2(g2, x23[j], a23[t]);
                        }
                    }
                }
        }
    }
#pragma unroll
    for (int c = 0; c < 4; ++c)
#pragma unroll
        for (int t = 0; t < 27; ++t) {
            float v = (c < 2 ? a01[t] : a23[t])[c & 1];
            v += __shfl_xor(v, 8); v += __shfl_xor(v, 16); v += __shfl_xor(v, 32);
            if ((threadIdx.x & 63) < 8) atomicAdd(&red[(quad * 4 + c) * 27 + t], v);
        }
    __syncthreads();
    for (int q = threadIdx.x; q < 864; q += 256) atomicAdd(&gw[q], red[q]);
}

static int c1_check(int B, int D, int H, int W) {
    if (!(B > 0 && D > 0 && H > 0 && W > 0)) return AZ_EINVAL;
    if (B > 65535 || D > 65535) return AZ_EUNSUPPORTED;
    return AZ_OK;
}

extern "C" int az_conv3d_c1_fwd(float *logits, const float *in, const float *w,
                                const float *addend, const float *in_scale, const float *in_shift, int B, int D,
                                int H, int W, void *stream) {
    AZ_REQUIRE_PTR(logits); AZ_REQUIRE_PTR(in); AZ_REQUIRE_PTR(w);
    if ((in_scale == nullptr) != (in_shift == nullptr)) return AZ_EINVAL;
    if (int e = c1_check(B, D, H, W)) return e;
    const int tiles_x = (W + C1F_TW - 1) / C1F_TW, tiles_y = (H + C1F_TH - 1) / C1F_TH;
    const int best = az_c1_fwd_dseg((long long)tiles_x * tiles_y * B, D);
    hipLaunchKernelGGL(c1_fwd_kernel, dim3(tiles_x * tiles_y, (D + best - 1) / best, B), dim3(256), 0,
                       az_stream(stream), logits, in, w, addend, in_scale, in_shift, D, H, W, tiles_x, best);
    return az_launch_status();
}

extern "C" int az_conv3d_c1_dgrad(float *grad_in, const float *grad_logits, const float *w,
                                  int B, int D, int H, int W, void *stream) {
    AZ_REQUIRE_PTR(grad_in); AZ_REQUIRE_PTR(grad_logits); AZ_REQUIRE_PTR(w);
    if (int e = c1_check(B, D, H, W)) return e;
    const int tiles_x = (W + C1_TW - 1) / C1_TW, tiles_y = (H + C1_TH - 1) / C1_TH;
    hipLaunchKernelGGL(c1_dgrad_kernel, dim3(tiles_x * tiles_y, D, B), dim3(256), 0,
                       az_stream(stream), grad_in, grad_logits, w, D, H, W, tiles_x);
    return az_launch_status();
}

extern "C" int az_conv3d_c1_wgrad(float *grad_w, const float *in, const float *grad_logits,
                                  const float *in_scale, const float *in_shift, int B, int D, int H, int W,
                                  void *stream) {
    AZ_REQUIRE_PTR(grad_w); AZ_REQUIRE_PTR(in); AZ_REQUIRE_PTR(grad_logits);
    if ((in_scale == nullptr) != (in_shift == nullptr)) return AZ_EINVAL;
    if (int e = c1_check(B, D, H, W)) return e;
    if (hipMemsetAsync(grad_w, 0, 864 * sizeof(float), az_stream(stream)) != hipSuccess)
        return AZ_ELAUNCH;
    const int tiles_x = (W + C1_TW - 1) / C1_TW, tiles_y = (H + C1_TH - 1) / C1_TH;
    const long long ntiles = az_c1_wgrad_tiles(B, D, H, W);
    const unsigned grid = (unsigned)az_c1_wgrad_grid(ntiles);
    hipLaunchKernelGGL(c1_wgrad_kernel, dim3(grid), dim3(256), 0, az_stream(stream), grad_w, in,
                       grad_logits, in_scale, in_shift, D, H, W, tiles_x, tiles_y, ntiles);
    return az_launch_status();
}

extern "C" int az_conv3d_c1_plan(long long *plan, int B, int D, int H, int W) {
    AZ_REQUIRE_PTR(plan);
    if (int e = c1_check(B, D, H, W)) return e;
    const long long patches = (long long)((W + C1F_TW - 1) / C1F_TW) * ((H + C1F_TH - 1) / C1F_TH) * B;
    const int dseg = az_c1_fwd_dseg(patches, D);
    const long long ntiles = az_c1_wgrad_tiles(B, D, H, W);
    plan[0] = dseg;
    plan[1] = patches * ((D + dseg - 1) / dseg);
    plan[2] = ntiles;
    plan[3] = az_c1_wgrad_grid(ntiles);
    return AZ_OK;
}
```

activezero_amd/csrc/az_launch_math.h:

```cpp
#pragma once
#if defined(__HIPCC__)
#define AZ_HD __host__ __device__ __forceinline__
#else
#define AZ_HD inline
#endif

AZ_HD int az_xcd_map(int bid, int nblk) {
    const int xcd = bid & 7, q8 = nblk >> 3, r8 = nblk & 7;
    return (xcd < r8 ? xcd * (q8 + 1) : r8 * (q8 + 1) + (xcd - r8) * q8) + (bid >> 3);
}

inline void az_roll_segments(long long patches, int Do, int forced, int &nseg, int &seg_len) {
    if (forced > 0) {
        seg_len = forced < Do ? forced : Do;
        nseg = (Do + seg_len - 1) / seg_len;
        return;
    }
    long long best = -1;
    nseg = 1; seg_len = Do;
    for (int n = 1; n <= Do; ++n) {
        const int len = (Do + n - 1) / n;
        const int nn = (Do + len - 1) / len;
        if (nn != n) continue;
        const long long rounds = (patches * n + 511) / 512;
        const long long cost = rounds * (len + 2) * 3 + 2;
        if (best < 0 || cost < best) { best = cost; nseg = n; seg_len = len; }
    }
}

inline void az_t2roll_segments(long long patches, int Di, int &nseg, int &seg_len) {
    long long best = -1;
    nseg = 1; seg_len = Di;
    for (int n = 1; n <= Di; ++n) {
        const int len = (Di + n - 1) / n;
        if ((Di + len - 1) / len != n) continue;
        const long long rounds = (patches * n + 255) / 256;
        const long long cost = rounds * (len * 4 + 2) + 1;
        if (best < 0 || cost < best) { best = cost; nseg = n; seg_len = len; }
    }
}

inline void az_s2roll_segments(long long patches, int Do, int forced, int &nseg, int &seg_len, int slots = 512) {
    if (forced > 0) {
        seg_len = forced < Do ? forced : Do;
        nseg = (Do + seg_len - 1) / seg_len;
        return;
    }
    long long best = -1;
    nseg = 1; seg_len = Do;
    for (int n = 1; n <= Do; ++n) {
        const int len = (Do + n - 1) / n;
        if ((Do + len - 1) / len != n) continue;
        const long long rounds = (patches * n + slots - 1) / slots;
        const long long cost = rounds * (27LL * len + 4 * (2 * len + 1) + 4);
        if (best < 0 || cost < best) { best = cost; nseg = n; seg_len = len; }
    }
}

inline void az_c2r_segments(long long patches, int N, int &nseg, int &seg_len) {
    long long best = -1;
    nseg = 1; seg_len = N;
    for (int n = 1; n <= N; ++n) {
        const int len = (N + n - 1) / n;
        if ((N + len - 1) / len != n) continue;
        const long long rounds = (patches * n + 511) / 512;
        const long long cost = rounds * (len * 3 + 2);
        if (best < 0 || cost < best) { best = cost; nseg = n; seg_len = len; }
    }
}

#define AZ_C1_FWD_SLOTS 768
inline long long az_c1_fwd_cost(long long patches, int D, int dseg) {
    const long long blocks = patches * ((D + dseg - 1) / dseg);
    return ((blocks + AZ_C1_FWD_SLOTS - 1) / AZ_C1_FWD_SLOTS) * (dseg + 2);
}
inline int az_c1_fwd_dseg(long long patches, int D) {
    int best = 1;
    long long best_cost = -1;
    for (int nseg = 1; nseg <= D; ++nseg) {
        const int dseg = (D + nseg - 1) / nseg;
        const long long cost = az_c1_fwd_cost(patches, D, dseg);
        if (best_cost < 0 || cost < best_cost) { best_cost = cost; best = dseg; }
    }
    return best;
}
#define AZ_C1_WGRAD_MAX_GRID 2048
inline long long az_c1_wgrad_tiles(int B, int D, int H, int W) {
    return (long long)B * D * ((H + 7) / 8) * ((W + 31) / 32);
}
inline int az_c1_wgrad_grid(long long ntiles) {
    return (int)(ntiles < AZ_C1_WGRAD_MAX_GRID ? ntiles : AZ_C1_WGRAD_MAX_GRID);
}

AZ_HD void az_roll_decode(int lin, int tiles_x, int tyb, int nseg, int &tix, int &tiy, int &seg, int &b) {
    tix = lin % tiles_x; lin /= tiles_x;
    tiy = lin % tyb; lin /= tyb;
    seg = lin % nseg;
    b = lin / nseg;
}

#define AZ_R_SY 10
#define AZ_R_SX 18
#define AZ_R_NQ (AZ_R_SY * AZ_R_SX * 8)
AZ_HD bool az_roll_piece(int tid, int it, int &sy, int &sx) {
    const int vox = (tid >> 3) + 32 * it;
    sy = vox / AZ_R_SX;
    sx = vox - sy * AZ_R_SX;
    return tid + 256 * it < AZ_R_NQ;
}

inline int az_wgrad16_workgroups(long long ncols, int slots, int ntiles, int cap) {
    int best = 1;
    double best_score = -1.0;
    const int step = 8 / (ntiles > 2 ? 4 : ntiles);
    for (int w = slots; w >= slots / 4 && w >= 1; w -= step) {
        if (w > ncols) continue;
        const long long per = (ncols + w - 1) / w;
        const double score = (double)ncols / (double)(per * slots);
        if (score > best_score + 1e-9) { best_score = score; best = w; }
    }
    if (ncols < slots / 4) best = (int)(ncols > 0 ? ncols : 1);
    if (cap > 0 && cap < best) best = cap;
    return best;
}

struct AzC2w16Plan { int seg_rows, nrseg, wgs; long long ncols; };
inline AzC2w16Plan az_c2w16_plan(int B, int H, int W, int slots) {
    const int nwchunk = (W + 15) / 16;
    AzC2w16Plan p{};
    p.nrseg = 1; p.wgs = 1;
    double best = -1.0;
    for (int nseg = 1; nseg <= 16; ++nseg) {
        int rows = (H + nseg - 1) / nseg;
        rows += rows & 1;
        const int segs = (H + rows - 1) / rows;
        const long long cols = (long long)B * nwchunk * segs;
        const int w = (int)(cols < slots ? cols : slots);
        const long long per = (cols + w - 1) / w;
        const double balance = (double)cols / (double)(per * w);
        const double occ = (double)w / (double)slots;
        const double amort = (double)rows / (double)(rows + 4);
        const double score = balance * (0.5 + 0.5 * occ) * amort;
        if (score > best) { best = score; p.nrseg = segs; p.wgs = w; p.seg_rows = rows; }
    }
    p.ncols = (long long)B * nwchunk * p.nrseg;
    return p;
}

struct AzC2wPlan { int blocks_per_combo, hseg_rows, nhseg; long long nitems; };
inline AzC2wPlan az_c2w_plan(int B, int H, int W, int mt, int nt, int ncombo, int ring_rows) {
    const int nwchunk = (W + 15) / 16;
    const int slots = 256 * 8 / (mt * nt);
    const int wq = (slots / ncombo) & ~7;
    const int wmax = wq > 8 ? wq : 8;
    const int wmin = wmax / 2 > 8 ? wmax / 2 : 8;
    const long long base_items = (long long)B * nwchunk;
    double best = -1.0;
    int best_w = 8, best_rows = H;
    for (int nseg = 1; nseg <= (H < 32 ? H : 32); ++nseg) {
        const int rows = (H + nseg - 1) / nseg;
        const int segs = (H + rows - 1) / rows;
        const long long items = base_items * segs;
        for (int w = wmax; w >= wmin; w -= 8) {
            const long long per = (items + w - 1) / w;
            const double balance = (double)items / (double)(per * w);
            const double occ = (double)w / (double)wmax;
            const double amort = (double)rows / (double)(rows + ring_rows - 1 + 2);
            const double score = balance * (0.5 + 0.5 * occ) * amort;
            if (score > best) { best = score; best_w = w; best_rows = rows; }
        }
    }
    AzC2wPlan p{};
    p.blocks_per_combo = best_w;
    p.hseg_rows = best_rows;
    p.nhseg = (H + best_rows - 1) / best_rows;
    p.nitems = base_items * p.nhseg;
    if (p.nitems < p.blocks_per_combo) p.blocks_per_combo = (int)((p.nitems + 7) & ~7LL);
    return p;
}

#define AZ_S2W_FPOS 17
#define AZ_S2W_FROWQ (AZ_S2W_FPOS * 8)
#define AZ_S2W_NFQ (3 * 8 * AZ_S2W_FROWQ)
#define AZ_S2W_RING 17
AZ_HD bool az_s2w_fine_piece(int f, int &pk, int &j, int &pp, int &lrow) {
    pk = f / (8 * AZ_S2W_FROWQ);
    const int g = f - pk * (8 * AZ_S2W_FROWQ);
    j = g / AZ_S2W_FROWQ;
    pp = (g - j * AZ_S2W_FROWQ) >> 3;
    lrow = (pp & 1) ? 9 + (pp >> 1) : (pp >> 1);
    return f < AZ_S2W_NFQ;
}
AZ_HD int az_s2w_tap_row(int kw) { return kw == 0 ? 0 : kw == 1 ? 9 : 1; }
AZ_HD int az_s2w_ring_slot(int fr) { return (fr + 1) % AZ_S2W_RING; }
AZ_HD void az_s2w_col_decode(long long col, int Dc, int nwchunk, int &cd, int &wc, int &b) {
    cd = (int)(col % Dc); col /= Dc;
    wc = (int)(col % nwchunk);
    b = (int)(col / nwchunk);
}

inline bool az_fits_buffer_offset(long long bytes) { return bytes > 0 && bytes < 0xffffff00LL; }
```

include/azhip.h:

```cpp
#ifndef AZHIP_H
#define AZHIP_H

#include <stddef.h>
#include <stdint.h>

#ifdef __cplusplus
extern "C" {
#endif

#define AZ_OK 0
#define AZ_EINVAL (-1)
#define AZ_ENULL (-2)
#define AZ_ELAUNCH (-3)
#define AZ_EUNSUPPORTED (-4)
#define AZ_EWORKSPACE (-5)

const char *az_strerror(int code);
#define AZ_ABI_VERSION 6
int az_abi_version(void);
int az_option(const char *name);
int az_hbm_copy_probe(float *dst, const float *src, long long n, void *stream);

int az_warp_scatter(float *dst, const float *src, const int32_t *disp, int N, int C, int H,
                    int W, int sign, void *stream);

int az_cost_volume_fwd(float *cost, const float *feat_l, const float *feat_r, int B, int C,
                       int d, int h, int w, void *stream);
int az_cost_volume_bwd(float *grad_l, float *grad_r, const float *grad_cost, int B, int C,
                       int d, int h, int w, void *stream);
int az_cost_volume_fwd_ndhwc(float *cost, const float *feat_l, const float *feat_r, int B,
                             int C, int d, int h, int w, void *stream);
int az_cost_volume_bwd_ndhwc(float *grad_l, float *grad_r, const float *grad_cost, int B,
                             int C, int d, int h, int w, void *stream);

int az_softargmin_fwd(float *disp_out, float *stats_out, const float *logits, int B, int d, int h,
                      int w, void *stream);
int az_softargmin_bwd(float *grad_logits, const float *grad_disp, const float *logits,
                      const float *stats, const float *disp_fwd, int B, int d, int h, int w,
                      void *stream);

int az_warp_gather_fwd(float *out, const float *img, const float *disp, int B, int C, int H,
                       int W, void *stream);
int az_warp_gather_bwd(float *grad_disp, float *grad_img, const float *grad_out,
                       const float *img, const float *disp, int B, int C, int H, int W,
                       void *stream);

int az_patch_reproj_fwd(double *acc, const float *L, const float *R, const float *disp,
                        const uint8_t *mask, int B, int C, int H, int W, int ps, float sign,
                        void *stream);
int az_patch_reproj_bwd(float *grad_disp, const float *grad_loss, const double *acc,
                        const float *L, const float *R, const float *disp, const uint8_t *mask,
                        int B, int C, int H, int W, int ps, float sign, void *stream);
int az_patch_reproj_vis(float *vis, const float *R, const float *disp, int B, int C, int H,
                        int W, int ps, float sign, void *stream);

int az_lcn(float *normed, float *stdv, const float *img, int B, int H, int W, int ksize,
           float eps, long long img_batch_stride, void *stream);


long long az_conv3d_packed_floats(int cin, int cout, int precision);
int az_conv3d_pack_weights(float *packed, const float *w, int cin, int cout,
                           long long stride_out, long long stride_in, int flip, int precision,
                           void *stream);
long long az_conv3d_num_tiles(int mode, int B, int Di, int Hi, int Wi);
long long az_conv3d_stats_tiles(int mode, int precision, int B, int cin, int cout, int Di, int Hi, int Wi);
int az_conv3d_fwd(float *out, const float *in, const float *in2, const float *packed_w,
                  const float *scale, const float *shift, const float *residual, int relu,
                  int mode, int src, int precision, int B, int cin, int cout, int Di, int Hi,
                  int Wi, void *stream);
int az_conv3d_fwd_stats(float *out, float *partials, float *counts, const float *in,
                        const float *in2, const float *packed_w, int mode, int src,
                        int precision, int B, int cin, int cout, int Di, int Hi, int Wi,
                        void *stream);
long long az_conv3d_wgrad_workspace(int cm, int cn);
int az_conv3d_wgrad(float *grad_w, float *workspace, long long workspace_bytes,
                    const float *coarse, const float *fine, int stride, int precision, int B,
                    int cm, int cn, int Dc, int Hc, int Wc, int Df, int Hf, int Wf, void *stream);

#define AZ_AMAX_SLOTS 16
#define AZ_AMAX_STRIDE 64
#define AZ_AMAX_FLOATS (AZ_AMAX_SLOTS * AZ_AMAX_STRIDE)
int az_absmax(float *amax, const float *x, long long n, void *stream);
#define AZ_PACK_2D_SAME 0
#define AZ_PACK_2D_ROLL 1
#define AZ_PACK_3D_GATHER 2
#define AZ_PACK_3D_ROLL 3
#define AZ_PACK_3D_ROLL2 4
typedef struct AzPackDesc {
    void *dst;
    const float *src;
    const float *amax;
    long long s_co, s_ci;
    int kind, cin, cout, ci_real, co_real, taps, flip, pad_;
} AzPackDesc;
int az_pack_f16_multi(const AzPackDesc *descs, const int *block_desc, const int *first_block, int nd, int nblocks,
                      void *stream);
typedef struct AzUnpackDesc {
    float *dst;
    const float *ws;
    int cm, cn, cm_real, cn_real, taps, pad_;
} AzUnpackDesc;
int az_wgrad_unpack_multi(const AzUnpackDesc *descs, const int *block_desc, const int *first_block, int nd, int nblocks,
                          void *stream);
long long az_conv3d_packed_floats_f16(int cin, int cout);
int az_conv3d_pack_weights_f16(float *packed, const float *w, const float *w_amax, int cin, int cout,
                               long long stride_out, long long stride_in, int flip, int mode, void *stream);
int az_conv3d_f16_layout(int mode, int cin, int cout);
int az_conv3d_fwd_f16_split_ok(int mode, int B, int cin, int cout, int Di, int Hi, int Wi);
int az_conv3d_wgrad_f16_split_ok(int stride, int B, int cm, int cn, int Dc, int Hc, int Wc, int Df, int Hf, int Wf);
int az_conv3d_fwd_f16(float *out, const float *in, const float *packed_w, const float *in_amax,
                      const float *w_amax, int in_split, const float *scale, const float *shift, const float *residual,
                      int relu, int mode, int B, int cin, int cout, int Di, int Hi, int Wi, void *stream);
long long az_conv3d_stats_tiles_f16(int mode, int B, int cin, int cout, int Di, int Hi, int Wi);
int az_conv3d_fwd_stats_f16(float *out, float *partials, float *counts, const float *in, const float *packed_w,
                            const float *in_amax, const float *w_amax, int mode, int B, int cin, int cout,
                            int Di, int Hi, int Wi, void *stream);
int az_conv3d_wgrad_f16(float *grad_w, float *workspace, long long workspace_bytes, const float *coarse,
                        const float *fine, const float *coarse_amax, const float *fine_amax, int split_mask, int stride,
                        int B, int cm, int cn, int Dc, int Hc, int Wc, int Df, int Hf, int Wf, void *stream);

int az_conv2d_pack_weights_f16(float *packed, const float *w, const float *w_amax, int cin, int cout,
                               int ci_real, int co_real, long long stride_out, long long stride_in, int kh,
                               int kw, int flip, void *stream);
int az_conv2d_fwd_f16(float *out, const float *in, const float *packed_w, const float *in_amax,
                      const float *w_amax, const float *scale, const float *shift, const float *residual,
                      int relu, int B, int H, int W, int cin, int cout, int in_cstride, int out_cstride,
                      int res_cstride, int kh, int kw, int dilation, void *stream);
int az_conv2d_fwd_stats_f16(float *out, float *partials, float *counts, const float *in, const float *packed_w,
                            const float *in_amax, const float *w_amax, int groups, int B, int H, int W,
                            int cin, int cout, int in_cstride, int out_cstride, int kh, int kw, int dilation,
                            void *stream);
int az_conv2d_pack_weights_bf16_flipped(float *packed, const float *w, int cin, int cout, long long stride_out,
                                        long long stride_in, int kh, int kw, void *stream);
int az_conv2d_wgrad_bf16(float *grad_w, float *workspace, long long workspace_bytes, const float *grad_out,
                         const float *in, int B, int H, int W, int cm, int cn, int cm_real, int cn_real,
                         int go_cstride, int in_cstride, void *stream);
int az_conv2d_wgrad_f16(float *grad_w, float *workspace, long long workspace_bytes, const float *grad_out,
                        const float *in, const float *go_amax, const float *in_amax, int B, int H, int W,
                        int cm, int cn, int cm_real, int cn_real, int go_cstride, int in_cstride, int kh,
                        int kw, int dilation, void *stream);
int az_conv2d_roll_pack_f16(float *packed, const float *w, const float *w_amax, int cin, int cout,
                            long long stride_out, long long stride_in, int flip, void *stream);
int az_conv2d_roll_fwd_f16(float *out, const float *in, const float *packed, const float *in_amax,
                           const float *w_amax, const float *scale, const float *shift, const float *residual,
                           int relu, int B, int H, int W, int cin, int cout, void *stream);
int az_conv2d_roll_fwd_stats_f16(float *out, float *partials, float *counts, const float *in, const float *packed,
                                 const float *in_amax, const float *w_amax, int groups, int B, int H, int W,
                                 int cin, int cout, void *stream);

int az_conv3d_c1_fwd(float *logits, const float *in, const float *w, const float *addend,
                     const float *in_scale, const float *in_shift, int B, int D, int H, int W, void *stream);
int az_conv3d_c1_dgrad(float *grad_in, const float *grad_logits, const float *w, int B, int D,
                       int H, int W, void *stream);
int az_conv3d_c1_wgrad(float *grad_w, const float *in, const float *grad_logits, const float *in_scale,
                       const float *in_shift, int B, int D, int H, int W, void *stream);
int az_conv3d_c1_plan(long long *plan , int B, int D, int H, int W);

long long az_bn3d_finalize_scratch(int C);
int az_bn3d_finalize(float *mean, float *invstd, float *scale, float *shift,
                     float *running_mean, float *running_var, const float *partials,
                     const float *counts, const float *gamma, const float *beta,
                     long long ntiles, int C, float eps, float momentum,
                     long long *num_batches_tracked, float *scratch, long long scratch_floats, void *stream);
long long az_bn3d_stats_tiles(long long nvox, int C);
int az_bn3d_stats(float *partials, float *counts, const float *x, long long nvox, int C, void *stream);
long long az_bn2d_workspace(int groups, long long nvox, int C);
int az_bn2d_fwd(float *y, float *mean, float *invstd, float *scale, float *shift, float *running_mean,
                float *running_var, const float *x, const float *residual, const float *gamma,
                const float *beta, float *workspace, long long workspace_bytes, int relu, int groups,
                long long nvox, int C, float eps, float momentum, long long *num_batches_tracked ,
                const float *partials, const float *counts, long long partial_tiles ,
                float *y_amax , void *stream);
int az_bn2d_bwd(float *dx, float *dz_out, float *dgamma, float *dbeta, float *workspace,
                long long workspace_bytes, const float *dy, const float *y, const float *x,
                const float *mean, const float *invstd, const float *gamma, const float *scale,
                const float *shift, int relu, int groups, long long nvox, int C,
                float *dx_amax , void *stream);
int az_bn3d_eval_affine(float *scale, float *shift, const float *gamma, const float *beta,
                        const float *running_mean, const float *running_var, float eps, int C,
                        void *stream);
int az_bn3d_apply(float *y, const float *x, const float *scale, const float *shift,
                  const float *residual, int relu, long long nvox, int C, float *y_amax, void *stream);
long long az_bn3d_bwd_workspace(long long nvox, int C);
int az_bn3d_bwd(float *dx, float *dz_out, float *dgamma, float *dbeta, float *coef,
                float *workspace, long long workspace_bytes, const float *dy, const float *y,
                const float *x, const float *mean, const float *invstd, const float *gamma,
                const float *scale, const float *shift, int relu, long long nvox, int C,
                float *dx_amax, int split_out, void *stream);
int az_spp_upsample_fwd(float *out, const float *in, int B, int hs, int ws, int H, int W, int C, int out_cstride,
                        void *stream);
long long az_spp_upsample_bwd_workspace(int B, int ws, int H, int C);
int az_spp_upsample_bwd(float *grad_in, float *workspace, long long workspace_bytes, const float *grad_out, int B,
                        int hs, int ws, int H, int W, int C, int gout_cstride, void *stream);
int az_add_relu(float *y, const float *a, const float *b, int relu, long long n, float *y_amax, void *stream);
int az_sum4(float *y, const float *a, const float *b, const float *c, const float *d, long long n,
            void *stream);

long long az_conv2d_packed_floats(int cin, int cout, int kh, int kw);
int az_conv2d_pack_weights(float *packed, const float *w, int cin, int cout, int ci_real, int co_real,
                           long long stride_out, long long stride_in, int kh, int kw, int flip,
                           void *stream);
int az_conv2d_fwd(float *out, const float *in, const float *packed_w, const float *scale,
                  const float *shift, const float *residual, int relu, int B, int H, int W, int cin,
                  int cout, int in_cstride, int out_cstride, int res_cstride, int kh, int kw,
                  int dilation, void *stream);
long long az_conv2d_wgrad_workspace(int cm, int cn, int kh, int kw);
int az_conv2d_wgrad(float *grad_w, float *workspace, long long workspace_bytes, const float *grad_out,
                    const float *in, int B, int H, int W, int cm, int cn, int cm_real, int cn_real,
                    int go_cstride, int in_cstride, int kh, int kw, int dilation, void *stream);
#define AZ_C2W_KERNEL_R16_AR0 0
#define AZ_C2W_KERNEL_R16_AR1 1
#define AZ_C2W_KERNEL_W64 2
#define AZ_C2W_KERNEL_GENERIC 3
int az_conv2d_wgrad_plan(long long *plan , int f16, int B, int H, int W, int cm, int cn, int kh, int kw, int dilation);
long long az_conv2d_stats_tiles(int B, int H, int W, int groups);
int az_conv2d_fwd_stats(float *out, float *partials, float *counts, const float *in, const float *packed_w,
                        int groups, int B, int H, int W, int cin, int cout, int in_cstride, int out_cstride,
                        int kh, int kw, int dilation, void *stream);

long long az_conv2d_roll_packed_floats(int cin, int cout);
int az_conv2d_roll_pack(float *packed, const float *w, int cin, int cout, long long stride_out, long long stride_in,
                        int flip, void *stream);
int az_conv2d_roll_fwd(float *out, const float *in, const float *packed, const float *scale, const float *shift,
                       const float *residual, int relu, int B, int H, int W, int cin, int cout, void *stream);
long long az_conv2d_roll_stats_rows(int groups, int B, int H, int W, int cin, int cout);
int az_conv2d_roll_fwd_stats(float *out, float *partials, float *counts, const float *in, const float *packed,
                             int groups, int B, int H, int W, int cin, int cout, void *stream);
int az_conv2d_pack_weights_bf16(float *packed, const float *w, int cin, int cout, long long stride_out,
                                long long stride_in, int kh, int kw, void *stream);
int az_conv2d_bf16_fwd(float *out, const float *in, const float *packed_w, const float *bias,
                       const float *residual, const float *gate_z, const float *gate_h, int act, int B, int H,
                       int W, int cin, int cout, int in_cstride, int out_cstride, int res_cstride,
                       int z_cstride, int h_cstride, void *stream);
int az_conv2d_pack_weights_h1(float *packed, const float *w, const float *w_amax, int cin, int cout, long long stride_out,
                              long long stride_in, int flip, void *stream);
int az_conv2d_h1_fwd(float *out, const float *in, const float *packed_w, const float *in_amax, const float *w_amax,
                     const float *bias, const float *residual, const float *gate_z, const float *gate_h, int act, int B, int H,
                     int W, int cin, int cout, int in_cstride, int out_cstride, int res_cstride, int z_cstride,
                     int h_cstride, void *stream);
int az_conv2d_wgrad_h1(float *grad_w, float *workspace, long long workspace_bytes, const float *grad_out, const float *in,
                       const float *go_amax, const float *in_amax, int B, int H, int W, int cm, int cn, int cm_real,
                       int cn_real, int go_cstride, int in_cstride, void *stream);
int az_rows_concat(float *dst, long long npix, long long hw, int nsrc, const float *const *srcs, const int *channels,
                   const int *kinds, void *stream);
int az_rows_slice_to_image(float *image, const float *rows, long long npix, long long hw, int ctot, int at, int c, void *stream);
int az_gru_rh(float *rhx, const float *zr, const float *hx, long long npix, int hid, int inp, void *stream);
int az_gru_out(float *hn, const float *zr, const float *q, const float *hx, long long npix, int hid, int inp, void *stream);
int az_gru_bwd1(float *dq_pre, float *dzr, float *dh_acc, const float *g, const float *zr, const float *q, const float *hx,
                long long npix, int hid, int inp, float *dq_amax, float *dzr_amax, void *stream);
int az_gru_bwd2(float *dzr, float *dh_acc, const float *d_rhx, const float *zr, const float *hx, long long npix, int hid, int inp,
                float *dzr_amax, void *stream);
int az_gru_bwd3(float *dh, float *dx, const float *dh_acc, const float *d_rhx, const float *d_hx, long long npix, int hid, int inp,
                void *stream);
int az_im2col_s2k3(float *patches, const float *x, int B, int C, int H, int W, int Kp, void *stream);
int az_col2im_s2k3(float *grad_x, const float *grad_patches, int B, int C, int H, int W, int Kp,
                   void *stream);

long long az_ir_pattern_workspace(int B, int H, int W, int ks);
int az_ir_pattern(float *pattern, float *workspace, long long workspace_bytes, const float *img_ir,
                  const float *img, int B, int H, int W, int ks, float threshold, void *stream);
int az_ir_pattern_mode(float *pattern, float *workspace, long long workspace_bytes, const float *img_ir,
                       const float *img, int B, int H, int W, int ks, float threshold, int mode, void *stream);

long long az_temporal_ir_workspace(int B, int T, int H, int W, int ks);
int az_temporal_ir(float *pattern, float *workspace, long long workspace_bytes, const void *stack,
                   int stack_is_u8, int B, int T, int H, int W, int ks, float threshold, void *stream);

int az_gt_from_right(float *disp_l, float *extra_l, float *keep_s, uint8_t *mask, int32_t *stats, const float *disp_r,
                     const float *extra, const float *keep, int N, int Ce, int Ck, int Hin, int Win, int H, int W,
                     float scale_h, float scale_w, float lo, float hi, void *stream);

int az_error_img(float *out, const float *est, const float *gt, const uint8_t *mask, int kind, float abs_thres,
                 float rel_thres, int layout, int B, int H, int W, void *stream);

long long az_augment_workspace(int B, int H, int W, int ks);
int az_augment(float *out, float *workspace, long long workspace_bytes, const void *img, int img_is_u8,
               const float *params, int B, int H, int W, int ks, int flags, void *stream);

int az_corr1d_volume(float *corr, const float *f1, const float *f2, int B, int C, int H, int W1,
                     int W2, void *stream);
int az_corr1d_volume_bwd(float *grad_f1, float *grad_f2, const float *grad_corr, const float *f1,
                         const float *f2, int B, int C, int H, int W1, int W2, void *stream);
int az_corr1d_pool(float *dst, const float *src, long long rows, int Wsrc, void *stream);
int az_corr1d_pool_bwd(float *grad_src, const float *grad_dst, long long rows, int Wsrc,
                       void *stream);
int az_corr1d_lookup_fwd(float *out, const float *pyr_level, const float *coords, int B, int H,
                         int W1, int W_level, int radius, int level, int ch_offset, int ch_total,
                         void *stream);
int az_corr1d_lookup_bwd(float *grad_pyr_level, const float *grad_out, const float *coords, int B,
                         int H, int W1, int W_level, int radius, int level, int ch_offset,
                         int ch_total, void *stream);
int az_corr1d_lookup_bwd_acc(float *grad_pyr_level, const float *grad_out, const float *coords, int B,
                         int H, int W1, int W_level, int radius, int level, int ch_offset,
                         int ch_total, void *stream);

int az_disp_loss_fwd(double *acc4, const float *pred3, const float *pred2, const float *pred1,
                     const float *gt, const unsigned char *mask, float lo, float hi, long long n,
                     void *stream);
int az_disp_loss_bwd(float *g3, float *g2, float *g1, const float *pred3, const float *pred2,
                     const float *pred1, const float *gt, const unsigned char *mask, float lo,
                     float hi, const float *gloss, const double *acc4, float w3, float w2, float w1,
                     long long n, void *stream);
int az_disp_metrics(double *acc8, const float *disp_gt, const float *depth_gt,
                    const float *disp_pred, const float *depth_pred, const float *focal_x_baseline,
                    const unsigned char *mask, int B, long long per_batch, void *stream);

int az_convex_up_fwd(float *up, const float *flow, const void *mask, int mask_f16, int N, int D, int D_out, int h,
                     int w, int factor, int mask_channels, int sign, void *stream);
long long az_convex_up_bwd_workspace(int N, int D_out, int h, int w);
int az_convex_up_bwd(void *g_mask, float *g_flow, void *workspace, long long workspace_bytes, const float *g_up,
                     const float *flow, const void *mask, int mask_f16, int N, int D, int D_out, int h, int w,
                     int factor, int mask_channels, int sign, void *stream);

int az_seq_loss_fwd(double *acc3, const float *pred, const float *gt, const void *valid, int valid_u8,
                    float max_flow, int tsign, long long n, void *stream);
int az_seq_loss_bwd(float *g_pred, const float *pred, const float *gt, const void *valid, int valid_u8,
                    float max_flow, int tsign, const float *gloss, const double *acc3, float weight, long long n,
                    void *stream);

int az_costconv_edge_width(int D, int W);
int az_costconv_num_classes(int D);
int az_costconv_merge_fwd(float *kl, float *kr, const float *weight, const float *ml, const float *mr, int ncls, void *stream);
int az_costconv_merge_bwd(float *grad_weight, const float *gkl, const float *gkr, const float *ml, const float *mr, int ncls,
                          void *stream);
int az_costconv_assemble_fwd(float *out, const float *F_bulk, const float *F_edge, const float *G, int B,
                             int D, int H, int W, void *stream);
int az_costconv_assemble_bwd(float *dF_bulk, float *dF_edge, float *dG, const float *grad_out, int B, int D,
                             int H, int W, void *stream);

#ifdef __cplusplus
}
#endif
#endif
```

Before: 47.41 pairs/s.

## Fuse logits-conv input gradient into the 32-channel BN backward for the head

In the cost-volume head, the 1-output-channel logits conv backward no longer materializes its input gradient. It parks the logits gradient and weight on the deferred affine object. The producing conv+BN backward then runs a new two-kernel head_bwd (reduce + apply) that recomputes the dgrad on the fly, applies the ReLU remask and BN backward, and writes dx directly. This removes a full-size 32-channel gradient tensor write and re-read in the largest activation. It adds cross-Function state passing via weak references and a non-materialized grad path, which is more fragile.

```diff
diff --git a/activezero_amd/conv3d.py b/activezero_amd/conv3d.py
--- a/activezero_amd/conv3d.py
+++ b/activezero_amd/conv3d.py
@@ -1,5 +1,6 @@
 import collections
 import os
+import weakref
 
 import torch
 
@@ -13,6 +14,7 @@
 _PREC = {"fp32": FP32, "bf16x6": BF16X6, "f16x3": F16X3}
 _BWD_F16 = os.environ.get("AZ_BWD_F16", "1") != "0"
 PRESPLIT = os.environ.get("AZ_PRESPLIT", "1") != "0"
+HEAD_BWD_FUSED = os.environ.get("AZ_HEAD_BWD_FUSED", "1") != "0"
 BF16X6_R16 = 2
 _ROLL = os.environ.get("AZ_CONV_ROLL", "1") != "0"
 
@@ -373,6 +375,8 @@
     @staticmethod
     def forward(ctx, x, weight, gamma, beta, residual, bn, mode, relu, arith, defer=None, x_slot=None, res_slot=None):
         ctx.x_slot, ctx.res_slot = x_slot, res_slot
+        ctx.set_materialize_grads(False)
+        ctx.head = None
         x = _chk(x, "x")
         if residual is not None:
             residual = _chk(residual, "residual")
@@ -408,6 +412,10 @@
             nvox = raw.numel() // cout
             if defer is not None and relu and residual is None:
                 defer.scale, defer.shift = scale, shift
+                _drop_parked()
+                if HEAD_BWD_FUSED and cout == 32 and mode == CONV_S1:
+                    defer.producer = True
+                    ctx.head = defer
                 y = raw
             else:
                 y = torch.empty_like(raw)
@@ -430,10 +438,18 @@
     def backward(ctx, gy):
         x, weight, gamma, raw, y, mean, invstd, scale, shift = ctx.saved_tensors
         mode, relu, has_res, cin, cout, arith, training = ctx.cfg
-        gy = _chk(gy.contiguous(), "grad_y")
+        parked = _take_parked(ctx.head)
+        if gy is not None:
+            gy = _chk(gy.contiguous(), "grad_y")
         nvox = raw.numel() // cout
-        with torch.cuda.device(gy.device):
-            gy = slot_leftover(ctx, gy)
+        with torch.cuda.device(raw.device):
+            if gy is not None or getattr(ctx, "az_out_slot", None) is not None and ctx.az_out_slot.parts:
+                gy = slot_leftover(ctx, gy if gy is not None else torch.zeros_like(raw))
+            if parked is not None and gy is not None:
+                gy = sum_parts([gy, _logits_input_grad(parked[0], parked[1], raw)])
+                parked = None
+            elif parked is None and gy is None:
+                gy = torch.zeros_like(raw)
             if not training:
                 s_, rm = invstd, mean
                 dz = gy * (y > 0).to(gy.dtype) if relu else gy
@@ -446,17 +462,27 @@
                 lib = _lib.lib()
                 dx_raw = torch.empty_like(raw)
                 dz = torch.empty_like(raw) if (has_res and relu) else None
-                dgamma, dbeta = gy.new_empty(cout), gy.new_empty(cout)
-                coef = gy.new_empty(cout, 3)
-                ws_bytes = lib.az_bn3d_bwd_workspace(nvox, cout)
-                ws = gy.new_empty(ws_bytes // 4)
-                dx_amax = gy.new_empty(AMAX_SLOTS) if arith.bwd16 else None
+                dgamma, dbeta = raw.new_empty(cout), raw.new_empty(cout)
+                coef = raw.new_empty(cout, 3)
+                dx_amax = raw.new_empty(AMAX_SLOTS) if arith.bwd16 else None
                 split = arith.bwd16 and PRESPLIT and _presplit_ok(x, raw, mode, cin, cout, ctx.needs_input_grad[0],
                                                                   ctx.needs_input_grad[1])
-                with profiler.scope(f"bn3d_bwd_{cout}", bytes=4.0 * raw.numel() * (7 if (relu and y is not None) else 5), bound="hbm"):
-                    _call("az_bn3d_bwd", _p(dx_raw), _p(dz), _p(dgamma), _p(dbeta), _p(coef), _p(ws), ws_bytes,
-                          _p(gy), _p(y), _p(raw), _p(mean), _p(invstd), _p(gamma.detach()), _p(scale), _p(shift),
-                          int(relu), nvox, cout, _p(dx_amax), int(split), _stream())
+                if parked is not None:
+                    g, w1 = parked
+                    b, d, h, wd, _ = raw.shape
+                    ws_bytes = lib.az_head_bwd_workspace(b, d, h, wd)
+                    ws = raw.new_empty(ws_bytes // 4)
+                    with profiler.scope("head_bwd_32", bytes=4.0 * raw.numel() * 3, bound="hbm"):
+                        _call("az_head_bwd", _p(dx_raw), _p(dgamma), _p(dbeta), _p(coef), _p(ws), ws_bytes, _p(g), _p(w1),
+                              _p(raw), _p(mean), _p(invstd), _p(gamma.detach()), _p(scale), _p(shift), b, d, h, wd,
+                              _p(dx_amax), int(split), _stream())
+                else:
+                    ws_bytes = lib.az_bn3d_bwd_workspace(nvox, cout)
+                    ws = gy.new_empty(ws_bytes // 4)
+                    with profiler.scope(f"bn3d_bwd_{cout}", bytes=4.0 * raw.numel() * (7 if (relu and y is not None) else 5), bound="hbm"):
+                        _call("az_bn3d_bwd", _p(dx_raw), _p(dz), _p(dgamma), _p(dbeta), _p(coef), _p(ws), ws_bytes,
+                              _p(gy), _p(y), _p(raw), _p(mean), _p(invstd), _p(gamma.detach()), _p(scale), _p(shift),
+                              int(relu), nvox, cout, _p(dx_amax), int(split), _stream())
                 if dx_amax is not None:
                     _set_amax(dx_raw, dx_amax)
                 if split:
@@ -479,10 +505,42 @@
 
     def __init__(self):
         self.scale = self.shift = None
+        self.producer = False
+        self.parked = None
 
     @property
     def pending(self):
         return self.scale is not None
+
+
+_PARKED = weakref.WeakSet()
+
+
+def _park(aff, g, w):
+    aff.parked = (g, w)
+    _PARKED.add(aff)
+
+
+def _take_parked(aff):
+    if aff is None or aff.parked is None:
+        return None
+    pair, aff.parked = aff.parked, None
+    _PARKED.discard(aff)
+    return pair
+
+
+def _drop_parked():
+    for aff in list(_PARKED):
+        aff.parked = None
+    _PARKED.clear()
+
+
+def _logits_input_grad(g, w, like):
+    b, d, h, wd, _ = _dims(like)
+    gx = torch.empty_like(like)
+    with profiler.scope("conv3d_c1_dgrad", bytes=4.0 * (gx.numel() + g.numel()), bound="hbm"):
+        _call("az_conv3d_c1_dgrad", _p(gx), _p(g), _p(w), b, d, h, wd, _stream())
+    return gx
 
 
 def conv_bn(x, conv, bn, mode, relu=False, residual=None, arith=None, defer=None):
@@ -509,8 +567,9 @@
 class _ConvLogits(torch.autograd.Function):
 
     @staticmethod
-    def forward(ctx, x, weight, addend, sink, scale=None, shift=None):
+    def forward(ctx, x, weight, addend, sink, scale=None, shift=None, park=None):
         ctx.sink = sink if (sink is not None and sink.owns(weight)) else None
+        ctx.park = park
         x = _chk(x, "x")
         w = _chk(weight.detach().contiguous(), "weight")
         b, d, h, wd, c = _dims(x)
@@ -534,20 +593,22 @@
         gx = gw = None
         with torch.cuda.device(g.device):
             if ctx.needs_input_grad[0]:
-                gx = torch.empty_like(x)
-                with profiler.scope("conv3d_c1_dgrad", bytes=4.0 * (x.numel() + g.numel()), bound="hbm"):
-                    _call("az_conv3d_c1_dgrad", _p(gx), _p(g), _p(w), b, d, h, wd, _stream())
+                if ctx.park is not None:
+                    _park(ctx.park, g, w)
+                else:
+                    gx = _logits_input_grad(g, w, x)
             if ctx.needs_input_grad[1]:
                 gw = torch.empty_like(w)
                 with overlap.scope(ctx.sink, x, g, gw, scale, shift), \
                         profiler.scope("conv3d_c1_wgrad", bytes=4.0 * (x.numel() + g.numel()), bound="hbm"):
                     _call("az_conv3d_c1_wgrad", _p(gw), _p(x), _p(g), _p(scale), _p(shift), b, d, h, wd, _stream())
-        return gx, gw, (g if ctx.has_add else None), None, None, None
+        return gx, gw, (g if ctx.has_add else None), None, None, None, None
 
 
 def conv_logits(x, conv, addend=None, sink=None, affine=None):
     sc, sh = (affine.scale, affine.shift) if (affine is not None and affine.pending) else (None, None)
-    return _ConvLogits.apply(x, sink.weight(conv.weight) if sink is not None else conv.weight, addend, sink, sc, sh)
+    park = affine if (sc is not None and affine.producer and x.grad_fn is not None and getattr(x.grad_fn, "head", None) is affine) else None
+    return _ConvLogits.apply(x, sink.weight(conv.weight) if sink is not None else conv.weight, addend, sink, sc, sh, park)
 
 
 class _AddRelu(torch.autograd.Function):
diff --git a/activezero_amd/csrc/az_bn3d.hip b/activezero_amd/csrc/az_bn3d.hip
--- a/activezero_amd/csrc/az_bn3d.hip
+++ b/activezero_amd/csrc/az_bn3d.hip
@@ -1,6 +1,6 @@
 #include <stdlib.h>
 
-#include "az_roll_common.h"
+#include "az_bn_bwd.h"
 
 __device__ __forceinline__ double bn_wave_sum(double v) {
 #pragma unroll
@@ -109,26 +109,6 @@
     shift[c] = beta[c] - rm[c] * sc;
 }
 
-typedef float az_v4f __attribute__((ext_vector_type(4)));
-template <bool NT>
-__device__ __forceinline__ float4 bn_ld4(const float4 *p) {
-    if (NT) {
-        const az_v4f v = __builtin_nontemporal_load(reinterpret_cast<const az_v4f *>(p));
-        return make_float4(v[0], v[1], v[2], v[3]);
-    }
-    return *p;
-}
-template <bool NT>
-__device__ __forceinline__ void bn_st4(float4 *p, const float4 &o) {
-    if (NT) {
-        const az_v4f v = {o.x, o.y, o.z, o.w};
-        __builtin_nontemporal_store(v, reinterpret_cast<az_v4f *>(p));
-    } else {
-        *p = o;
-    }
-}
-#define BN_NT_BYTES (256LL << 20)
-
 template <int C, bool NT>
 __global__ void __launch_bounds__(256)
 bn_apply_kernel(float4 *__restrict__ y, const float4 *__restrict__ x,
@@ -277,7 +257,6 @@
     }
 }
 
-#define BN_BWD_PARTIAL_FLOATS 32768
 template <int C, bool NT>
 __global__ void __launch_bounds__(256)
 bn_bwd_apply_kernel(float4 *__restrict__ dx, float4 *__restrict__ dz_out,
@@ -290,8 +269,7 @@
                     unsigned *__restrict__ amax = nullptr, const unsigned *__restrict__ pmax = nullptr) {
     constexpr int C4 = C / 4;
     unsigned am = 0;
-    float split_scale = 1.f;
-    __shared__ float smu[C], sis[C], k0[C], k1[C], k2[C], ssc[C], ssh[C];
+    __shared__ BnBwdShared<C> sm;
     const bool remask = relu && scale != nullptr;
     const int grp = blockIdx.y;
     {
@@ -300,103 +278,26 @@
         mean += grp * C; invstd += grp * C; coef += grp * C * 3;
         if (remask) { scale += grp * C; shift += grp * C; }
     }
-    if (remask && threadIdx.x < C) { ssc[threadIdx.x] = scale[threadIdx.x]; ssh[threadIdx.x] = shift[threadIdx.x]; }
-    if (threadIdx.x < C) {
-        smu[threadIdx.x] = mean[threadIdx.x];
-        sis[threadIdx.x] = invstd[threadIdx.x];
-    }
-    constexpr int COLS = C / 2, ROWS = 256 / COLS;
-    static_assert(COLS <= 64 && 64 % COLS == 0, "a partial row must tile a wave");
-    __shared__ float wsum[4][2 * C];
-    const int j = threadIdx.x % COLS, r = threadIdx.x / COLS, wave = threadIdx.x >> 6;
-    const bool writer = blockIdx.x == 0;
-    const int g_lo = (writer && grp == 0) ? 0 : grp, g_hi = (writer && grp == 0) ? (int)gridDim.y : grp + 1;
-    double dg_tot = 0.0, db_tot = 0.0;
-    for (int g = g_lo; g < g_hi; ++g) {
-        const float4 *p4 = reinterpret_cast<const float4 *>(partial) + (size_t)g * nblocks * COLS;
-        double a0 = 0.0, a1 = 0.0, a2 = 0.0, a3 = 0.0;
-        for (int blk = r; blk < nblocks; blk += ROWS) {
-            const float4 v = p4[(size_t)blk * COLS + j];
-            a0 += v.x; a1 += v.y; a2 += v.z; a3 += v.w;
-        }
-#pragma unroll
-        for (int off = COLS; off < 64; off <<= 1) {
-            a0 += __shfl_xor(a0, off); a1 += __shfl_xor(a1, off); a2 += __shfl_xor(a2, off); a3 += __shfl_xor(a3, off);
-        }
-        __syncthreads();
-        if ((threadIdx.x & 63) < COLS) {
-            wsum[wave][4 * j + 0] = (float)a0; wsum[wave][4 * j + 1] = (float)a1;
-            wsum[wave][4 * j + 2] = (float)a2; wsum[wave][4 * j + 3] = (float)a3;
-        }
-        __syncthreads();
-        if (threadIdx.x < C) {
-            const int c = threadIdx.x;
-            const double sa = ((double)wsum[0][2 * c] + (double)wsum[1][2 * c]) + ((double)wsum[2][2 * c] + (double)wsum[3][2 * c]);
-            const double sb = ((double)wsum[0][2 * c + 1] + (double)wsum[1][2 * c + 1]) + ((double)wsum[2][2 * c + 1] + (double)wsum[3][2 * c + 1]);
-            db_tot += sa; dg_tot += sb;
-            if (g == grp) {
-                k0[c] = gamma[c] * sis[c];
-                k1[c] = (float)(sa / nvox);
-                k2[c] = (float)(sb / nvox);
-                if (writer) { coef[c * 3 + 0] = k0[c]; coef[c * 3 + 1] = k1[c]; coef[c * 3 + 2] = k2[c]; }
-            }
-        }
-    }
-    if (writer && grp == 0 && threadIdx.x < C) { dbeta[threadIdx.x] = (float)db_tot; dgamma[threadIdx.x] = (float)dg_tot; }
-    if (pmax) {
-        const uint4 *m4 = reinterpret_cast<const uint4 *>(pmax);
-        uint4 m = make_uint4(0, 0, 0, 0);
-        for (int blk = r; blk < nblocks; blk += ROWS) {
-            const uint4 v = m4[(size_t)blk * COLS + j];
-            m.x = max(m.x, v.x); m.y = max(m.y, v.y); m.z = max(m.z, v.z); m.w = max(m.w, v.w);
-        }
-#pragma unroll
-        for (int off = COLS; off < 64; off <<= 1) {
-            m.x = max(m.x, (unsigned)__shfl_xor((int)m.x, off)); m.y = max(m.y, (unsigned)__shfl_xor((int)m.y, off));
-            m.z = max(m.z, (unsigned)__shfl_xor((int)m.z, off)); m.w = max(m.w, (unsigned)__shfl_xor((int)m.w, off));
-        }
-        __syncthreads();
-        if ((threadIdx.x & 63) < COLS) {
-            wsum[wave][4 * j + 0] = __uint_as_float(m.x); wsum[wave][4 * j + 1] = __uint_as_float(m.y);
-            wsum[wave][4 * j + 2] = __uint_as_float(m.z); wsum[wave][4 * j + 3] = __uint_as_float(m.w);
-        }
-        __syncthreads();
-        float bnd = 0.f;
-        if (threadIdx.x < C) {
-            const int c = threadIdx.x;
-            const float gm = fmaxf(fmaxf(wsum[0][2 * c], wsum[1][2 * c]), fmaxf(wsum[2][2 * c], wsum[3][2 * c]));
-            const float xm = fmaxf(fmaxf(wsum[0][2 * c + 1], wsum[1][2 * c + 1]), fmaxf(wsum[2][2 * c + 1], wsum[3][2 * c + 1]));
-            bnd = fabsf(k0[c]) * (gm + fabsf(k1[c]) + xm * fabsf(k2[c])) * 1.000001f;
-            bnd = bnd < __builtin_inff() ? bnd : 0.f;
-        }
-#pragma unroll
-        for (int off = 32; off > 0; off >>= 1) bnd = fmaxf(bnd, __shfl_xor(bnd, off));
-        __shared__ float bwave[4];
-        if ((threadIdx.x & 63) == 0) bwave[wave] = bnd;
-        __syncthreads();
-        bnd = fmaxf(fmaxf(bwave[0], bwave[1]), fmaxf(bwave[2], bwave[3]));
-        split_scale = az_pow2(az_f16_scale_exp(bnd));
-        if (writer && grp == 0 && threadIdx.x == 0 && amax) amax[0] = __float_as_uint(bnd);
-    }
-    __syncthreads();
+    const float split_scale = bn_bwd_prologue<C>(sm, mean, invstd, coef, scale, shift, remask, partial, nblocks, gamma, dgamma,
+                                                 dbeta, nvox, amax, pmax, grp, (int)gridDim.y, blockIdx.x == 0);
     for (long long i = blockIdx.x * 256LL + threadIdx.x; i < total4; i += gridDim.x * 256LL) {
         const int c = (int)(i % C4) * 4;
         float4 g = bn_ld4<NT>(&dy[i]);
         const float4 xx = bn_ld4<NT>(&x[i]);
         if (relu) {
             float4 yy;
-            if (remask) yy = make_float4(fmaf(xx.x, ssc[c + 0], ssh[c + 0]), fmaf(xx.y, ssc[c + 1], ssh[c + 1]),
-                                         fmaf(xx.z, ssc[c + 2], ssh[c + 2]), fmaf(xx.w, ssc[c + 3], ssh[c + 3]));
+            if (remask) yy = make_float4(fmaf(xx.x, sm.ssc[c + 0], sm.ssh[c + 0]), fmaf(xx.y, sm.ssc[c + 1], sm.ssh[c + 1]),
+                                         fmaf(xx.z, sm.ssc[c + 2], sm.ssh[c + 2]), fmaf(xx.w, sm.ssc[c + 3], sm.ssh[c + 3]));
             else yy = bn_ld4<NT>(&y[i]);
             g.x = yy.x > 0.f ? g.x : 0.f; g.y = yy.y > 0.f ? g.y : 0.f;
             g.z = yy.z > 0.f ? g.z : 0.f; g.w = yy.w > 0.f ? g.w : 0.f;
         }
         if (dz_out) bn_st4<NT>(&dz_out[i], g);
         float4 o;
-        o.x = k0[c + 0] * (g.x - k1[c + 0] - (xx.x - smu[c + 0]) * sis[c + 0] * k2[c + 0]);
-        o.y = k0[c + 1] * (g.y - k1[c + 1] - (xx.y - smu[c + 1]) * sis[c + 1] * k2[c + 1]);
-        o.z = k0[c + 2] * (g.z - k1[c + 2] - (xx.z - smu[c + 2]) * sis[c + 2] * k2[c + 2]);
-        o.w = k0[c + 3] * (g.w - k1[c + 3] - (xx.w - smu[c + 3]) * sis[c + 3] * k2[c + 3]);
+        o.x = bn_bwd_dx(g.x, xx.x, sm.smu[c + 0], sm.sis[c + 0], sm.k0[c + 0], sm.k1[c + 0], sm.k2[c + 0]);
+        o.y = bn_bwd_dx(g.y, xx.y, sm.smu[c + 1], sm.sis[c + 1], sm.k0[c + 1], sm.k1[c + 1], sm.k2[c + 1]);
+        o.z = bn_bwd_dx(g.z, xx.z, sm.smu[c + 2], sm.sis[c + 2], sm.k0[c + 2], sm.k1[c + 2], sm.k2[c + 2]);
+        o.w = bn_bwd_dx(g.w, xx.w, sm.smu[c + 3], sm.sis[c + 3], sm.k0[c + 3], sm.k1[c + 3], sm.k2[c + 3]);
         if (pmax) {
             bn_st4<NT>(&dx[i], az_presplit_f16x4(make_float4(o.x * split_scale, o.y * split_scale, o.z * split_scale, o.w * split_scale)));
         } else {
diff --git a/activezero_amd/csrc/az_bn_bwd.h b/activezero_amd/csrc/az_bn_bwd.h
--- /dev/null
+++ b/activezero_amd/csrc/az_bn_bwd.h
@@ -0,0 +1,123 @@
+#pragma once
+#include "az_roll_common.h"
+
+typedef float az_v4f __attribute__((ext_vector_type(4)));
+template <bool NT>
+__device__ __forceinline__ float4 bn_ld4(const float4 *p) {
+    if (NT) {
+        const az_v4f v = __builtin_nontemporal_load(reinterpret_cast<const az_v4f *>(p));
+        return make_float4(v[0], v[1], v[2], v[3]);
+    }
+    return *p;
+}
+template <bool NT>
+__device__ __forceinline__ void bn_st4(float4 *p, const float4 &o) {
+    if (NT) {
+        const az_v4f v = {o.x, o.y, o.z, o.w};
+        __builtin_nontemporal_store(v, reinterpret_cast<az_v4f *>(p));
+    } else {
+        *p = o;
+    }
+}
+#define BN_NT_BYTES (256LL << 20)
+
+#define BN_BWD_PARTIAL_FLOATS 32768
+
+template <int C>
+struct __attribute__((aligned(16))) BnBwdShared {
+    float smu[C], sis[C], k0[C], k1[C], k2[C], ssc[C], ssh[C];
+    float wsum[4][2 * C];
+    float bwave[4];
+};
+
+template <int C>
+__device__ __forceinline__ float bn_bwd_prologue(BnBwdShared<C> &sm, const float *__restrict__ mean,
+                                                 const float *__restrict__ invstd, float *__restrict__ coef,
+                                                 const float *__restrict__ scale, const float *__restrict__ shift,
+                                                 bool remask, const float *__restrict__ partial, int nblocks,
+                                                 const float *__restrict__ gamma, float *__restrict__ dgamma,
+                                                 float *__restrict__ dbeta, double nvox, unsigned *__restrict__ amax,
+                                                 const unsigned *__restrict__ pmax, int grp, int ngroups, bool writer) {
+    float split_scale = 1.f;
+    if (remask && threadIdx.x < C) { sm.ssc[threadIdx.x] = scale[threadIdx.x]; sm.ssh[threadIdx.x] = shift[threadIdx.x]; }
+    if (threadIdx.x < C) {
+        sm.smu[threadIdx.x] = mean[threadIdx.x];
+        sm.sis[threadIdx.x] = invstd[threadIdx.x];
+    }
+    constexpr int COLS = C / 2, ROWS = 256 / COLS;
+    static_assert(COLS <= 64 && 64 % COLS == 0, "a partial row must tile a wave");
+    const int j = threadIdx.x % COLS, r = threadIdx.x / COLS, wave = threadIdx.x >> 6;
+    const int g_lo = (writer && grp == 0) ? 0 : grp, g_hi = (writer && grp == 0) ? ngroups : grp + 1;
+    double dg_tot = 0.0, db_tot = 0.0;
+    for (int g = g_lo; g < g_hi; ++g) {
+        const float4 *p4 = reinterpret_cast<const float4 *>(partial) + (size_t)g * nblocks * COLS;
+        double a0 = 0.0, a1 = 0.0, a2 = 0.0, a3 = 0.0;
+        for (int blk = r; blk < nblocks; blk += ROWS) {
+            const float4 v = p4[(size_t)blk * COLS + j];
+            a0 += v.x; a1 += v.y; a2 += v.z; a3 += v.w;
+        }
+#pragma unroll
+        for (int off = COLS; off < 64; off <<= 1) {
+            a0 += __shfl_xor(a0, off); a1 += __shfl_xor(a1, off); a2 += __shfl_xor(a2, off); a3 += __shfl_xor(a3, off);
+        }
+        __syncthreads();
+        if ((threadIdx.x & 63) < COLS) {
+            sm.wsum[wave][4 * j + 0] = (float)a0; sm.wsum[wave][4 * j + 1] = (float)a1;
+            sm.wsum[wave][4 * j + 2] = (float)a2; sm.wsum[wave][4 * j + 3] = (float)a3;
+        }
+        __syncthreads();
+        if (threadIdx.x < C) {
+            const int c = threadIdx.x;
+            const double sa = ((double)sm.wsum[0][2 * c] + (double)sm.wsum[1][2 * c]) + ((double)sm.wsum[2][2 * c] + (double)sm.wsum[3][2 * c]);
+            const double sb = ((double)sm.wsum[0][2 * c + 1] + (double)sm.wsum[1][2 * c + 1]) + ((double)sm.wsum[2][2 * c + 1] + (double)sm.wsum[3][2 * c + 1]);
+            db_tot += sa; dg_tot += sb;
+            if (g == grp) {
+                sm.k0[c] = gamma[c] * sm.sis[c];
+                sm.k1[c] = (float)(sa / nvox);
+                sm.k2[c] = (float)(sb / nvox);
+                if (writer) { coef[c * 3 + 0] = sm.k0[c]; coef[c * 3 + 1] = sm.k1[c]; coef[c * 3 + 2] = sm.k2[c]; }
+            }
+        }
+    }
+    if (writer && grp == 0 && threadIdx.x < C) { dbeta[threadIdx.x] = (float)db_tot; dgamma[threadIdx.x] = (float)dg_tot; }
+    if (pmax) {
+        const uint4 *m4 = reinterpret_cast<const uint4 *>(pmax);
+        uint4 m = make_uint4(0, 0, 0, 0);
+        for (int blk = r; blk < nblocks; blk += ROWS) {
+            const uint4 v = m4[(size_t)blk * COLS + j];
+            m.x = max(m.x, v.x); m.y = max(m.y, v.y); m.z = max(m.z, v.z); m.w = max(m.w, v.w);
+        }
+#pragma unroll
+        for (int off = COLS; off < 64; off <<= 1) {
+            m.x = max(m.x, (unsigned)__shfl_xor((int)m.x, off)); m.y = max(m.y, (unsigned)__shfl_xor((int)m.y, off));
+            m.z = max(m.z, (unsigned)__shfl_xor((int)m.z, off)); m.w = max(m.w, (unsigned)__shfl_xor((int)m.w, off));
+        }
+        __syncthreads();
+        if ((threadIdx.x & 63) < COLS) {
+            sm.wsum[wave][4 * j + 0] = __uint_as_float(m.x); sm.wsum[wave][4 * j + 1] = __uint_as_float(m.y);
+            sm.wsum[wave][4 * j + 2] = __uint_as_float(m.z); sm.wsum[wave][4 * j + 3] = __uint_as_float(m.w);
+        }
+        __syncthreads();
+        float bnd = 0.f;
+        if (threadIdx.x < C) {
+            const int c = threadIdx.x;
+            const float gm = fmaxf(fmaxf(sm.wsum[0][2 * c], sm.wsum[1][2 * c]), fmaxf(sm.wsum[2][2 * c], sm.wsum[3][2 * c]));
+            const float xm = fmaxf(fmaxf(sm.wsum[0][2 * c + 1], sm.wsum[1][2 * c + 1]), fmaxf(sm.wsum[2][2 * c + 1], sm.wsum[3][2 * c + 1]));
+            bnd = fabsf(sm.k0[c]) * (gm + fabsf(sm.k1[c]) + xm * fabsf(sm.k2[c])) * 1.000001f;
+            bnd = bnd < __builtin_inff() ? bnd : 0.f;
+        }
+#pragma unroll
+        for (int off = 32; off > 0; off >>= 1) bnd = fmaxf(bnd, __shfl_xor(bnd, off));
+        if ((threadIdx.x & 63) == 0) sm.bwave[wave] = bnd;
+        __syncthreads();
+        bnd = fmaxf(fmaxf(sm.bwave[0], sm.bwave[1]), fmaxf(sm.bwave[2], sm.bwave[3]));
+        split_scale = az_pow2(az_f16_scale_exp(bnd));
+        if (writer && grp == 0 && threadIdx.x == 0 && amax) amax[0] = __float_as_uint(bnd);
+    }
+    __syncthreads();
+    return split_scale;
+}
+
+__device__ __forceinline__ float bn_bwd_dx(float g, float x, float mu, float is, float k0, float k1, float k2) {
+    return k0 * (g - k1 - (x - mu) * is * k2);
+}
diff --git a/activezero_amd/csrc/az_c1_tile.h b/activezero_amd/csrc/az_c1_tile.h
--- /dev/null
+++ b/activezero_amd/csrc/az_c1_tile.h
@@ -0,0 +1,78 @@
+#pragma once
+#include "az_common.h"
+
+#define C1_TH 8
+#define C1_TW 32
+#define C1_VS 36
+#define C1_GP 36
+typedef float c1_f2 __attribute__((ext_vector_type(2)));
+#define C1_FMA2(a, b, c) __builtin_elementwise_fma(a, b, c)
+
+__device__ __forceinline__ void c1_load_gtile(float *gt, const float *__restrict__ gout, int b,
+                                              int od, int ty0, int tx0, int D, int H, int W) {
+    constexpr int SX = C1_TW + 2, SY = C1_TH + 2;
+    for (int q = threadIdx.x; q < 3 * SY * SX; q += 256) {
+        const int sx = q % SX;
+        const int r = q / SX;
+        const int sy = r % SY, sd = r / SY;
+        const int gd = od - 1 + sd, gh = ty0 - 1 + sy, gw = tx0 - 1 + sx;
+        gt[r * C1_GP + sx] = (gd >= 0 && gd < D && gh >= 0 && gh < H && gw >= 0 && gw < W)
+                                 ? gout[(((size_t)b * D + gd) * H + gh) * W + gw] : 0.f;
+    }
+}
+#define C1_GT_PER_THREAD 4
+__device__ __forceinline__ void c1_fetch_gtile(float (&pre)[C1_GT_PER_THREAD], const float *__restrict__ gout, int b,
+                                               int od, int ty0, int tx0, int D, int H, int W) {
+    constexpr int SX = C1_TW + 2, SY = C1_TH + 2;
+    static_assert(C1_GT_PER_THREAD * 256 >= 3 * SY * SX, "a thread's pieces must cover the tile");
+#pragma unroll
+    for (int i = 0; i < C1_GT_PER_THREAD; ++i) {
+        const int q = threadIdx.x + 256 * i;
+        const int sx = q % SX;
+        const int r = q / SX;
+        const int sy = r % SY, sd = r / SY;
+        const int gd = od - 1 + sd, gh = ty0 - 1 + sy, gw = tx0 - 1 + sx;
+        pre[i] = (q < 3 * SY * SX && gd >= 0 && gd < D && gh >= 0 && gh < H && gw >= 0 && gw < W)
+                     ? gout[(((size_t)b * D + gd) * H + gh) * W + gw] : 0.f;
+    }
+}
+__device__ __forceinline__ void c1_store_gtile(float *gt, const float (&pre)[C1_GT_PER_THREAD]) {
+    constexpr int SX = C1_TW + 2, SY = C1_TH + 2;
+#pragma unroll
+    for (int i = 0; i < C1_GT_PER_THREAD; ++i) {
+        const int q = threadIdx.x + 256 * i;
+        if (q < 3 * SY * SX) gt[(q / SX) * C1_GP + q % SX] = pre[i];
+    }
+}
+
+__device__ __forceinline__ void c1_dgrad_acc8(c1_f2 (&acc)[8], const float *gt, const c1_f2 (&wp)[27], int ly, int lx0) {
+    constexpr int SY = C1_TH + 2;
+#pragma unroll
+    for (int j = 0; j < 8; ++j) acc[j] = c1_f2{0.f, 0.f};
+#pragma unroll
+    for (int kd = 0; kd < 3; ++kd)
+#pragma unroll
+        for (int kh = 0; kh < 3; ++kh) {
+            float r[12];
+            {
+                const float *row = static_cast<const float *>(__builtin_assume_aligned(
+                    gt + ((2 - kd) * SY + ly + 2 - kh) * C1_GP + lx0, 16));
+                const float4 a = *reinterpret_cast<const float4 *>(row);
+                const float4 c = *reinterpret_cast<const float4 *>(row + 4);
+                const float2 e = *reinterpret_cast<const float2 *>(row + 8);
+                r[0] = a.x; r[1] = a.y; r[2] = a.z; r[3] = a.w; r[4] = c.x; r[5] = c.y; r[6] = c.z; r[7] = c.w;
+                r[8] = e.x; r[9] = e.y;
+            }
+#pragma unroll
+            for (int kw = 0; kw < 3; ++kw) {
+                const int t = (kd * 3 + kh) * 3 + kw;
+#pragma unroll
+                for (int j = 0; j < 8; ++j) {
+                    const c1_f2 g2 = {r[j + 2 - kw], r[j + 2 - kw]};
+                    acc[j] = C1_FMA2(g2, wp[t], acc[j]);
+                }
+            }
+        }
+#pragma unroll
+    for (int j = 0; j < 8; ++j) asm volatile("" : "+v"(acc[j]));
+}
diff --git a/activezero_amd/csrc/az_conv3d_c1.hip b/activezero_amd/csrc/az_conv3d_c1.hip
--- a/activezero_amd/csrc/az_conv3d_c1.hip
+++ b/activezero_amd/csrc/az_conv3d_c1.hip
@@ -1,13 +1,5 @@
-#include "az_common.h"
+#include "az_c1_tile.h"
 #include "az_launch_math.h"
-
-#define C1_TH 8
-#define C1_TW 32
-#define C1_VS 36
-#define C1_GP 36
-typedef float c1_f2 __attribute__((ext_vector_type(2)));
-#define C1_FMA2(a, b, c) __builtin_elementwise_fma(a, b, c)
-
 
 #define C1F_TH 8
 #define C1F_TW 16
@@ -116,18 +108,6 @@
     }
 }
 
-__device__ __forceinline__ void c1_load_gtile(float *gt, const float *__restrict__ gout, int b,
-                                              int od, int ty0, int tx0, int D, int H, int W) {
-    constexpr int SX = C1_TW + 2, SY = C1_TH + 2;
-    for (int q = threadIdx.x; q < 3 * SY * SX; q += 256) {
-        const int sx = q % SX;
-        const int r = q / SX;
-        const int sy = r % SY, sd = r / SY;
-        const int gd = od - 1 + sd, gh = ty0 - 1 + sy, gw = tx0 - 1 + sx;
-        gt[r * C1_GP + sx] = (gd >= 0 && gd < D && gh >= 0 && gh < H && gw >= 0 && gw < W)
-                                 ? gout[(((size_t)b * D + gd) * H + gh) * W + gw] : 0.f;
-    }
-}
 __device__ __forceinline__ void c1_row6(float (&r)[6], const float *gt, int pd, int sy, int lx0) {
     const float *row = static_cast<const float *>(__builtin_assume_aligned(gt + (pd * (C1_TH + 2) + sy) * C1_GP + lx0, 16));
     const float4 a = *reinterpret_cast<const float4 *>(row);
@@ -153,34 +133,7 @@
         const int gi = p * 16 + grp, ly = gi >> 2, lx0 = (gi & 3) * 8;
         const int oh = ty0 + ly;
         c1_f2 acc[8];
-#pragma unroll
-        for (int j = 0; j < 8; ++j) acc[j] = c1_f2{0.f, 0.f};
-#pragma unroll
-        for (int kd = 0; kd < 3; ++kd)
-#pragma unroll
-            for (int kh = 0; kh < 3; ++kh) {
-                float r[12];
-                {
-                    const float *row = static_cast<const float *>(__builtin_assume_aligned(
-                        gt + ((2 - kd) * SY + ly + 2 - kh) * C1_GP + lx0, 16));
-                    const float4 a = *reinterpret_cast<const float4 *>(row);
-                    const float4 c = *reinterpret_cast<const float4 *>(row + 4);
-                    const float2 e = *reinterpret_cast<const float2 *>(row + 8);
-                    r[0] = a.x; r[1] = a.y; r[2] = a.z; r[3] = a.w; r[4] = c.x; r[5] = c.y; r[6] = c.z; r[7] = c.w;
-                    r[8] = e.x; r[9] = e.y;
-                }
-#pragma unroll
-                for (int kw = 0; kw < 3; ++kw) {
-                    const int t = (kd * 3 + kh) * 3 + kw;
-#pragma unroll
-                    for (int j = 0; j < 8; ++j) {
-                        const c1_f2 g2 = {r[j + 2 - kw], r[j + 2 - kw]};
-                        acc[j] = C1_FMA2(g2, wp[t], acc[j]);
-                    }
-                }
-            }
-#pragma unroll
-        for (int j = 0; j < 8; ++j) asm volatile("" : "+v"(acc[j]));
+        c1_dgrad_acc8(acc, gt, wp, ly, lx0);
         if (oh < H) {
             float *dst = gin + ((((size_t)b * D + od) * H + oh) * W + tx0 + lx0) * 32 + cp * 2;
 #pragma unroll
diff --git a/activezero_amd/csrc/az_head_bwd.hip b/activezero_amd/csrc/az_head_bwd.hip
--- /dev/null
+++ b/activezero_amd/csrc/az_head_bwd.hip
@@ -0,0 +1,271 @@
+#include "az_bn_bwd.h"
+#include "az_c1_tile.h"
+#include "az_launch_math.h"
+
+static_assert(AZ_HEAD_BWD_ROWS * 32 * 2 == BN_BWD_PARTIAL_FLOATS, "the reduce pass's rows must fit the apply prologue's bound");
+
+template <int BANKS>
+__device__ __forceinline__ float head_swap8(float keep, float send) {
+    return __builtin_bit_cast(float, __builtin_amdgcn_update_dpp(__builtin_bit_cast(int, keep), __builtin_bit_cast(int, send),
+                                                                 0x128, 0xf, BANKS, false));
+}
+__device__ __forceinline__ void head_quads(float4 (&g)[4], const c1_f2 (&acc)[8]) {
+#pragma unroll
+    for (int j = 0; j < 4; ++j) {
+        g[j].x = head_swap8<0xC>(acc[j][0], acc[4 + j][0]);
+        g[j].y = head_swap8<0xC>(acc[j][1], acc[4 + j][1]);
+        g[j].z = head_swap8<0x3>(acc[4 + j][0], acc[j][0]);
+        g[j].w = head_swap8<0x3>(acc[4 + j][1], acc[j][1]);
+    }
+}
+__device__ __forceinline__ void head_weights(c1_f2 (&wp)[27], const float *__restrict__ w, int cp) {
+    const int pair = 2 * (cp & 7) + (cp >> 3);
+#pragma unroll
+    for (int t = 0; t < 27; ++t) wp[t] = c1_f2{w[(pair * 2 + 0) * 27 + t], w[(pair * 2 + 1) * 27 + t]};
+}
+__device__ __forceinline__ float4 head_mask(const float4 &g, const float4 &xx, const float4 &sc, const float4 &sh) {
+    const float4 yy = make_float4(fmaf(xx.x, sc.x, sh.x), fmaf(xx.y, sc.y, sh.y), fmaf(xx.z, sc.z, sh.z), fmaf(xx.w, sc.w, sh.w));
+    return make_float4(yy.x > 0.f ? g.x : 0.f, yy.y > 0.f ? g.y : 0.f, yy.z > 0.f ? g.z : 0.f, yy.w > 0.f ? g.w : 0.f);
+}
+
+template <bool NT>
+__global__ void __launch_bounds__(256)
+head_bwd_reduce_kernel(float *__restrict__ partial, unsigned *__restrict__ pmax, unsigned *__restrict__ amax_zero,
+                       const float *__restrict__ gout, const float *__restrict__ w, const float *__restrict__ raw,
+                       const float *__restrict__ mean, const float *__restrict__ invstd,
+                       const float *__restrict__ scale, const float *__restrict__ shift, int D, int H, int W,
+                       int tiles_x, int tiles_y, long long nitems) {
+    constexpr int SY = C1_TH + 2;
+    __shared__ __attribute__((aligned(16))) float gt[3 * SY * C1_GP];
+    if (amax_zero && blockIdx.x == 0 && threadIdx.x < AZ_AMAX_SLOTS) amax_zero[threadIdx.x * AZ_AMAX_STRIDE] = 0u;
+    const int cp = threadIdx.x & 15, grp = threadIdx.x >> 4, quad = cp & 7, half = cp >> 3;
+    c1_f2 wp[27];
+    head_weights(wp, w, cp);
+    const float4 sc = reinterpret_cast<const float4 *>(scale)[quad], sh = reinterpret_cast<const float4 *>(shift)[quad];
+    const float4 mu = reinterpret_cast<const float4 *>(mean)[quad], is = reinterpret_cast<const float4 *>(invstd)[quad];
+    const float4 zero4 = make_float4(0.f, 0.f, 0.f, 0.f);
+    float4 s1 = zero4, s2 = zero4;
+    uint4 mg = make_uint4(0, 0, 0, 0), mx = make_uint4(0, 0, 0, 0);
+    float pre[C1_GT_PER_THREAD];
+    int tix, tiy, od, b;
+    az_head_bwd_decode(blockIdx.x, tiles_x, tiles_y, D, tix, tiy, od, b);
+    c1_fetch_gtile(pre, gout, b, od, tiy * C1_TH, tix * C1_TW, D, H, W);
+    for (long long item = blockIdx.x; item < nitems; item += gridDim.x) {
+        az_head_bwd_decode(item, tiles_x, tiles_y, D, tix, tiy, od, b);
+        const int tx0 = tix * C1_TW, ty0 = tiy * C1_TH;
+        __syncthreads();
+        c1_store_gtile(gt, pre);
+        __syncthreads();
+        if (item + gridDim.x < nitems) {
+            int nx, ny, nd, nb;
+            az_head_bwd_decode(item + gridDim.x, tiles_x, tiles_y, D, nx, ny, nd, nb);
+            c1_fetch_gtile(pre, gout, nb, nd, ny * C1_TH, nx * C1_TW, D, H, W);
+        }
+        float4 i1 = zero4, i2 = zero4;
+#pragma unroll 1
+        for (int p = 0; p < C1_TH * C1_TW / 128; ++p) {
+            const int gi = p * 16 + grp, ly = gi >> 2, lx0 = (gi & 3) * 8;
+            const int oh = ty0 + ly, ow0 = tx0 + lx0 + 4 * half;
+            const float4 *src = reinterpret_cast<const float4 *>(raw) + ((((size_t)b * D + od) * H + oh) * W + ow0) * 8 + quad;
+            float4 xx[4];
+#pragma unroll
+            for (int j = 0; j < 4; ++j) xx[j] = (oh < H && ow0 + j < W) ? bn_ld4<NT>(src + j * 8) : zero4;
+            c1_f2 acc[8];
+            c1_dgrad_acc8(acc, gt, wp, ly, lx0);
+            float4 g[4];
+            head_quads(g, acc);
+            float4 t1[4], t2[4];
+#pragma unroll
+            for (int j = 0; j < 4; ++j) {
+                const bool ok = oh < H && ow0 + j < W;
+                const float4 dz = head_mask(g[j], xx[j], sc, sh);
+                const float4 xh = make_float4((xx[j].x - mu.x) * is.x, (xx[j].y - mu.y) * is.y, (xx[j].z - mu.z) * is.z, (xx[j].w - mu.w) * is.w);
+                t1[j] = ok ? dz : zero4;
+                t2[j] = ok ? make_float4(dz.x * xh.x, dz.y * xh.y, dz.z * xh.z, dz.w * xh.w) : zero4;
+                if (pmax && ok) {
+                    mg.x = max(mg.x, az_finite_abs_bits(dz.x)); mg.y = max(mg.y, az_finite_abs_bits(dz.y));
+                    mg.z = max(mg.z, az_finite_abs_bits(dz.z)); mg.w = max(mg.w, az_finite_abs_bits(dz.w));
+                    mx.x = max(mx.x, az_finite_abs_bits(xh.x)); mx.y = max(mx.y, az_finite_abs_bits(xh.y));
+                    mx.z = max(mx.z, az_finite_abs_bits(xh.z)); mx.w = max(mx.w, az_finite_abs_bits(xh.w));
+                }
+            }
+            i1.x += (t1[0].x + t1[1].x) + (t1[2].x + t1[3].x); i1.y += (t1[0].y + t1[1].y) + (t1[2].y + t1[3].y);
+            i1.z += (t1[0].z + t1[1].z) + (t1[2].z + t1[3].z); i1.w += (t1[0].w + t1[1].w) + (t1[2].w + t1[3].w);
+            i2.x += (t2[0].x + t2[1].x) + (t2[2].x + t2[3].x); i2.y += (t2[0].y + t2[1].y) + (t2[2].y + t2[3].y);
+            i2.z += (t2[0].z + t2[1].z) + (t2[2].z + t2[3].z); i2.w += (t2[0].w + t2[1].w) + (t2[2].w + t2[3].w);
+        }
+        s1.x += i1.x; s1.y += i1.y; s1.z += i1.z; s1.w += i1.w;
+        s2.x += i2.x; s2.y += i2.y; s2.z += i2.z; s2.w += i2.w;
+    }
+#pragma unroll
+    for (int off = 8; off < 64; off <<= 1) {
+        s1.x += __shfl_xor(s1.x, off); s1.y += __shfl_xor(s1.y, off); s1.z += __shfl_xor(s1.z, off); s1.w += __shfl_xor(s1.w, off);
+        s2.x += __shfl_xor(s2.x, off); s2.y += __shfl_xor(s2.y, off); s2.z += __shfl_xor(s2.z, off); s2.w += __shfl_xor(s2.w, off);
+    }
+    __shared__ float4 r1[4][8], r2[4][8];
+    const int wave = threadIdx.x >> 6, lane = threadIdx.x & 63;
+    if (lane < 8) { r1[wave][lane] = s1; r2[wave][lane] = s2; }
+    __syncthreads();
+    if (threadIdx.x < 8) {
+        const float4 a0 = r1[0][quad], a1 = r1[1][quad], a2 = r1[2][quad], a3 = r1[3][quad];
+        const float4 b0 = r2[0][quad], b1 = r2[1][quad], b2 = r2[2][quad], b3 = r2[3][quad];
+        float *p = partial + ((size_t)blockIdx.x * 32 + quad * 4) * 2;
+        p[0] = (a0.x + a1.x) + (a2.x + a3.x); p[1] = (b0.x + b1.x) + (b2.x + b3.x);
+        p[2] = (a0.y + a1.y) + (a2.y + a3.y); p[3] = (b0.y + b1.y) + (b2.y + b3.y);
+        p[4] = (a0.z + a1.z) + (a2.z + a3.z); p[5] = (b0.z + b1.z) + (b2.z + b3.z);
+        p[6] = (a0.w + a1.w) + (a2.w + a3.w); p[7] = (b0.w + b1.w) + (b2.w + b3.w);
+    }
+    if (pmax) {
+#pragma unroll
+        for (int off = 8; off < 64; off <<= 1) {
+            mg.x = max(mg.x, (unsigned)__shfl_xor((int)mg.x, off)); mg.y = max(mg.y, (unsigned)__shfl_xor((int)mg.y, off));
+            mg.z = max(mg.z, (unsigned)__shfl_xor((int)mg.z, off)); mg.w = max(mg.w, (unsigned)__shfl_xor((int)mg.w, off));
+            mx.x = max(mx.x, (unsigned)__shfl_xor((int)mx.x, off)); mx.y = max(mx.y, (unsigned)__shfl_xor((int)mx.y, off));
+            mx.z = max(mx.z, (unsigned)__shfl_xor((int)mx.z, off)); mx.w = max(mx.w, (unsigned)__shfl_xor((int)mx.w, off));
+        }
+        __syncthreads();
+        uint4 (*q1)[8] = reinterpret_cast<uint4 (*)[8]>(r1), (*q2)[8] = reinterpret_cast<uint4 (*)[8]>(r2);
+        if (lane < 8) { q1[wave][lane] = mg; q2[wave][lane] = mx; }
+        __syncthreads();
+        if (threadIdx.x < 8) {
+#pragma unroll
+            for (int k = 1; k < 4; ++k) {
+                const uint4 a = q1[k][quad], c = q2[k][quad];
+                mg.x = max(mg.x, a.x); mg.y = max(mg.y, a.y); mg.z = max(mg.z, a.z); mg.w = max(mg.w, a.w);
+                mx.x = max(mx.x, c.x); mx.y = max(mx.y, c.y); mx.z = max(mx.z, c.z); mx.w = max(mx.w, c.w);
+            }
+            unsigned *p = pmax + ((size_t)blockIdx.x * 32 + quad * 4) * 2;
+            p[0] = mg.x; p[1] = mx.x; p[2] = mg.y; p[3] = mx.y;
+            p[4] = mg.z; p[5] = mx.z; p[6] = mg.w; p[7] = mx.w;
+        }
+    }
+}
+
+template <bool NT>
+__global__ void __launch_bounds__(256)
+head_bwd_apply_kernel(float *__restrict__ dx, float *__restrict__ coef, float *__restrict__ dgamma,
+                      float *__restrict__ dbeta, unsigned *__restrict__ amax, const unsigned *__restrict__ pmax,
+                      const float *__restrict__ partial, int nblocks, const float *__restrict__ gout,
+                      const float *__restrict__ w, const float *__restrict__ raw, const float *__restrict__ mean,
+                      const float *__restrict__ invstd, const float *__restrict__ gamma,
+                      const float *__restrict__ scale, const float *__restrict__ shift, double nvox, int D, int H, int W,
+                      int tiles_x, int tiles_y, long long nitems) {
+    constexpr int SY = C1_TH + 2;
+    __shared__ __attribute__((aligned(16))) float gt[3 * SY * C1_GP];
+    __shared__ BnBwdShared<32> sm;
+    unsigned am = 0;
+    const int cp = threadIdx.x & 15, grp = threadIdx.x >> 4, quad = cp & 7, half = cp >> 3;
+    float pre[C1_GT_PER_THREAD];
+    int tix, tiy, od, b;
+    az_head_bwd_decode(blockIdx.x, tiles_x, tiles_y, D, tix, tiy, od, b);
+    c1_fetch_gtile(pre, gout, b, od, tiy * C1_TH, tix * C1_TW, D, H, W);
+    const float split_scale = bn_bwd_prologue<32>(sm, mean, invstd, coef, scale, shift, true, partial, nblocks, gamma, dgamma,
+                                                  dbeta, nvox, amax, pmax, 0, 1, blockIdx.x == 0);
+    c1_f2 wp[27];
+    head_weights(wp, w, cp);
+    const float4 zero4 = make_float4(0.f, 0.f, 0.f, 0.f);
+    for (long long item = blockIdx.x; item < nitems; item += gridDim.x) {
+        az_head_bwd_decode(item, tiles_x, tiles_y, D, tix, tiy, od, b);
+        const int tx0 = tix * C1_TW, ty0 = tiy * C1_TH;
+        __syncthreads();
+        c1_store_gtile(gt, pre);
+        __syncthreads();
+        if (item + gridDim.x < nitems) {
+            int nx, ny, nd, nb;
+            az_head_bwd_decode(item + gridDim.x, tiles_x, tiles_y, D, nx, ny, nd, nb);
+            c1_fetch_gtile(pre, gout, nb, nd, ny * C1_TH, nx * C1_TW, D, H, W);
+        }
+#pragma unroll 1
+        for (int p = 0; p < C1_TH * C1_TW / 128; ++p) {
+            const int gi = p * 16 + grp, ly = gi >> 2, lx0 = (gi & 3) * 8;
+            const int oh = ty0 + ly, ow0 = tx0 + lx0 + 4 * half;
+            const size_t at = ((((size_t)b * D + od) * H + oh) * W + ow0) * 8 + quad;
+            const float4 *src = reinterpret_cast<const float4 *>(raw) + at;
+            float4 xx[4];
+#pragma unroll
+            for (int j = 0; j < 4; ++j) xx[j] = (oh < H && ow0 + j < W) ? bn_ld4<NT>(src + j * 8) : zero4;
+            c1_f2 acc[8];
+            c1_dgrad_acc8(acc, gt, wp, ly, lx0);
+            float4 g[4];
+            head_quads(g, acc);
+            const float4 sc = *reinterpret_cast<const float4 *>(&sm.ssc[quad * 4]), sh = *reinterpret_cast<const float4 *>(&sm.ssh[quad * 4]);
+            const float4 mu = *reinterpret_cast<const float4 *>(&sm.smu[quad * 4]), is = *reinterpret_cast<const float4 *>(&sm.sis[quad * 4]);
+            const float4 k0 = *reinterpret_cast<const float4 *>(&sm.k0[quad * 4]), k1 = *reinterpret_cast<const float4 *>(&sm.k1[quad * 4]);
+            const float4 k2 = *reinterpret_cast<const float4 *>(&sm.k2[quad * 4]);
+            float4 *dst = reinterpret_cast<float4 *>(dx) + at;
+#pragma unroll
+            for (int j = 0; j < 4; ++j) {
+                if (!(oh < H && ow0 + j < W)) continue;
+                const float4 dz = head_mask(g[j], xx[j], sc, sh);
+                float4 o;
+                o.x = bn_bwd_dx(dz.x, xx[j].x, mu.x, is.x, k0.x, k1.x, k2.x);
+                o.y = bn_bwd_dx(dz.y, xx[j].y, mu.y, is.y, k0.y, k1.y, k2.y);
+                o.z = bn_bwd_dx(dz.z, xx[j].z, mu.z, is.z, k0.z, k1.z, k2.z);
+                o.w = bn_bwd_dx(dz.w, xx[j].w, mu.w, is.w, k0.w, k1.w, k2.w);
+                if (pmax) {
+                    bn_st4<NT>(dst + j * 8, az_presplit_f16x4(make_float4(o.x * split_scale, o.y * split_scale, o.z * split_scale, o.w * split_scale)));
+                } else {
+                    bn_st4<NT>(dst + j * 8, o);
+                    az_amax_acc(am, o);
+                }
+            }
+        }
+    }
+    if (amax && !pmax) az_amax_flush(amax, am);
+}
+
+static int head_check(int B, int D, int H, int W) {
+    if (!(B > 0 && D > 0 && H > 0 && W > 0)) return AZ_EINVAL;
+    if (B > 65535 || D > 65535) return AZ_EUNSUPPORTED;
+    return AZ_OK;
+}
+
+extern "C" long long az_head_bwd_workspace(int B, int D, int H, int W) {
+    if (int e = head_check(B, D, H, W)) return e;
+    return az_head_bwd_workspace_bytes(az_head_bwd_items(B, D, H, W));
+}
+
+extern "C" int az_head_bwd(float *dx, float *dgamma, float *dbeta, float *coef, float *workspace,
+                           long long workspace_bytes, const float *grad_logits, const float *w, const float *raw,
+                           const float *mean, const float *invstd, const float *gamma, const float *scale,
+                           const float *shift, int B, int D, int H, int W, float *dx_amax, int split_out, void *stream) {
+    unsigned *const am = reinterpret_cast<unsigned *>(dx_amax);
+    AZ_REQUIRE_PTR(dx); AZ_REQUIRE_PTR(dgamma); AZ_REQUIRE_PTR(dbeta); AZ_REQUIRE_PTR(coef);
+    AZ_REQUIRE_PTR(workspace); AZ_REQUIRE_PTR(grad_logits); AZ_REQUIRE_PTR(w); AZ_REQUIRE_PTR(raw);
+    AZ_REQUIRE_PTR(mean); AZ_REQUIRE_PTR(invstd); AZ_REQUIRE_PTR(gamma); AZ_REQUIRE_PTR(scale); AZ_REQUIRE_PTR(shift);
+    if (int e = head_check(B, D, H, W)) return e;
+    const long long items = az_head_bwd_items(B, D, H, W);
+    if (workspace_bytes < az_head_bwd_workspace_bytes(items)) return AZ_EWORKSPACE;
+    if (split_out && !am) return AZ_ENULL;
+    const int tiles_x = (W + C1_TW - 1) / C1_TW, tiles_y = (H + C1_TH - 1) / C1_TH;
+    const int rows = az_head_bwd_grid(items), agrid = az_head_bwd_apply_grid(items);
+    const long long nvox = (long long)B * D * H * W;
+    unsigned *const pmax = split_out ? reinterpret_cast<unsigned *>(workspace) + (size_t)rows * 32 * 2 : nullptr;
+    hipStream_t s = az_stream(stream);
+    if (nvox * 32 * 4 >= BN_NT_BYTES) {
+        hipLaunchKernelGGL(head_bwd_reduce_kernel<true>, dim3(rows), dim3(256), 0, s, workspace, pmax, am, grad_logits, w, raw,
+                           mean, invstd, scale, shift, D, H, W, tiles_x, tiles_y, items);
+        hipLaunchKernelGGL(head_bwd_apply_kernel<true>, dim3(agrid), dim3(256), 0, s, dx, coef, dgamma, dbeta, am,
+                           (const unsigned *)pmax, (const float *)workspace, rows, grad_logits, w, raw, mean, invstd, gamma,
+                           scale, shift, (double)nvox, D, H, W, tiles_x, tiles_y, items);
+    } else {
+        hipLaunchKernelGGL(head_bwd_reduce_kernel<false>, dim3(rows), dim3(256), 0, s, workspace, pmax, am, grad_logits, w, raw,
+                           mean, invstd, scale, shift, D, H, W, tiles_x, tiles_y, items);
+        hipLaunchKernelGGL(head_bwd_apply_kernel<false>, dim3(agrid), dim3(256), 0, s, dx, coef, dgamma, dbeta, am,
+                           (const unsigned *)pmax, (const float *)workspace, rows, grad_logits, w, raw, mean, invstd, gamma,
+                           scale, shift, (double)nvox, D, H, W, tiles_x, tiles_y, items);
+    }
+    return az_launch_status();
+}
+
+extern "C" int az_head_bwd_plan(long long *plan, int B, int D, int H, int W) {
+    AZ_REQUIRE_PTR(plan);
+    if (int e = head_check(B, D, H, W)) return e;
+    const long long items = az_head_bwd_items(B, D, H, W);
+    const int grid = az_head_bwd_grid(items);
+    plan[0] = items;
+    plan[1] = grid;
+    plan[2] = (items + grid - 1) / grid;
+    plan[3] = az_head_bwd_apply_grid(items);
+    return AZ_OK;
+}
diff --git a/activezero_amd/csrc/az_launch_math.h b/activezero_amd/csrc/az_launch_math.h
--- a/activezero_amd/csrc/az_launch_math.h
+++ b/activezero_amd/csrc/az_launch_math.h
@@ -90,6 +90,22 @@
 }
 inline int az_c1_wgrad_grid(long long ntiles) {
     return (int)(ntiles < AZ_C1_WGRAD_MAX_GRID ? ntiles : AZ_C1_WGRAD_MAX_GRID);
+}
+#define AZ_HEAD_BWD_ROWS 512
+#define AZ_HEAD_BWD_APPLY_MAX_GRID 768
+inline long long az_head_bwd_items(int B, int D, int H, int W) { return az_c1_wgrad_tiles(B, D, H, W); }
+inline int az_head_bwd_grid(long long items) { return (int)(items < AZ_HEAD_BWD_ROWS ? items : AZ_HEAD_BWD_ROWS); }
+inline int az_head_bwd_apply_grid(long long items) {
+    return (int)(items < AZ_HEAD_BWD_APPLY_MAX_GRID ? items : AZ_HEAD_BWD_APPLY_MAX_GRID);
+}
+inline long long az_head_bwd_workspace_bytes(long long items) {
+    return 2LL * az_head_bwd_grid(items) * 32 * 2 * (long long)sizeof(float);
+}
+AZ_HD void az_head_bwd_decode(long long item, int tiles_x, int tiles_y, int D, int &tix, int &tiy, int &od, int &b) {
+    tix = (int)(item % tiles_x); item /= tiles_x;
+    tiy = (int)(item % tiles_y); item /= tiles_y;
+    od = (int)(item % D);
+    b = (int)(item / D);
 }
 
 AZ_HD void az_roll_decode(int lin, int tiles_x, int tyb, int nseg, int &tix, int &tiy, int &seg, int &b) {
diff --git a/include/azhip.h b/include/azhip.h
--- a/include/azhip.h
+++ b/include/azhip.h
@@ -187,6 +187,12 @@
                 const float *x, const float *mean, const float *invstd, const float *gamma,
                 const float *scale, const float *shift, int relu, long long nvox, int C,
                 float *dx_amax, int split_out, void *stream);
+long long az_head_bwd_workspace(int B, int D, int H, int W);
+int az_head_bwd(float *dx, float *dgamma, float *dbeta, float *coef, float *workspace, long long workspace_bytes,
+                const float *grad_logits, const float *w, const float *raw, const float *mean, const float *invstd,
+                const float *gamma, const float *scale, const float *shift, int B, int D, int H, int W,
+                float *dx_amax, int split_out, void *stream);
+int az_head_bwd_plan(long long *plan , int B, int D, int H, int W);
 int az_spp_upsample_fwd(float *out, const float *in, int B, int hs, int ws, int H, int W, int C, int out_cstride,
                         void *stream);
 long long az_spp_upsample_bwd_workspace(int B, int ws, int H, int C);
```

Measured after the change: 47.74 pairs/s (median of 6 runs). Within noise of the previous version (+0.7%).
